# modelscope/FunASR

Hardware: AMD Instinct MI355X
Metric: audio-seconds/sec (RTF^-1) Paraformer-large 30s@bs64 (higher is better)
Workload: dtype f32 (GEMM / self-attention operands split into 2 fp16 planes, 3 fp16 MFMA products, f32 accumulate; all else f32)

## Files before the change

### funasr_amd/_lib.py

```python
from __future__ import annotations

import ctypes as C
import os
import subprocess
import threading

_HERE = os.path.dirname(os.path.abspath(__file__))
LIB_PATH = os.environ.get("PF_LIB_PATH") or os.path.join(_HERE, "libparaformer_hip.so")
CSRC_DIR = os.path.join(_HERE, "csrc")

ABI_VERSION = 5

_lock = threading.Lock()
_lib = None


class HipRuntimeError(RuntimeError):
    """A pf_* entry point returned a non-zero status."""


class pf_frontend_config(C.Structure):
    _fields_ = [
        ("sample_rate", C.c_int32), ("frame_length", C.c_int32), ("frame_shift", C.c_int32),
        ("n_mels", C.c_int32), ("lfr_m", C.c_int32), ("lfr_n", C.c_int32),
# ... 186 lines not shown
    "pf_conformer_set_tensor": (C.c_int, [_vp, C.c_char_p, _vp, _i64]),
    "pf_conformer_missing": (C.c_int, [_vp]),
    "pf_conformer_set_precision": (C.c_int, [_vp, _i32]),
    "pf_conformer_num_frames": (_i32, [_vp, _i32, _i32]),
    "pf_conformer_forward": (C.c_int, [_vp, _vp, _pi32, _i32, _i32, _vp, _pi32, _vp]),
    "pf_tfencoder_create": (_vp, [C.POINTER(pf_tfencoder_config)]),
    "pf_tfencoder_destroy": (None, [_vp]),
    "pf_tfencoder_set_tensor": (C.c_int, [_vp, C.c_char_p, _vp, _i64]),
    "pf_tfencoder_missing": (C.c_int, [_vp]),
    "pf_tfencoder_set_precision": (C.c_int, [_vp, _i32]),
    "pf_tfencoder_num_frames": (_i32, [_vp, _i32, _i32]),
    "pf_tfencoder_forward": (C.c_int, [_vp, _vp, _pi32, _i32, _i32, _vp, _pi32, _vp]),
    "pf_k_tf_attention": (C.c_int, [_vp, _vp, _i32, _i32, _i32, _vp, _vp]),
    "pf_k_tf_embed_rows": (C.c_int, [_vp, _i32, _vp, _i32, _i32, _i32, _f32, _vp, _vp]),
    "pf_tdecoder_create": (_vp, [C.POINTER(pf_tdecoder_config)]),
    "pf_tdecoder_destroy": (None, [_vp]),
    "pf_tdecoder_set_tensor": (C.c_int, [_vp, C.c_char_p, _vp, _i64]),
    "pf_tdecoder_missing": (C.c_int, [_vp]),
    "pf_tdecoder_begin": (C.c_int, [_vp, _vp, _i32, _i32, _i32, _vp]),
    "pf_tdecoder_step": (C.c_int, [_vp, _pi32, _i32, _i32, _vp, _vp]),
    "pf_tdecoder_reorder": (C.c_int, [_vp, _pi32, _i32, _vp]),
    "pf_fsmndecoder_create": (_vp, [C.POINTER(pf_fsmndecoder_config)]),
    "pf_fsmndecoder_destroy": (None, [_vp]),
    "pf_fsmndecoder_set_tensor": (C.c_int, [_vp, C.c_char_p, _vp, _i64]),
    "pf_fsmndecoder_missing": (C.c_int, [_vp]),
    "pf_fsmndecoder_begin": (C.c_int, [_vp, _vp, _i32, _i32, _i32, _vp]),
    "pf_fsmndecoder_step": (C.c_int, [_vp, _pi32, _i32, _i32, _vp, _vp]),
    "pf_fsmndecoder_reorder": (C.c_int, [_vp, _pi32, _i32, _vp]),
    "pf_k_fsmn_step": (C.c_int, [_vp, _vp, _vp, _vp, _vp, _vp, _vp, _vp, _i32, _i32, _i32, _i32, _i32, _vp, _vp, _f32, _vp, _vp, _vp]),
    "pf_k_cross_attention_step": (C.c_int, [_vp, _vp, _i32, _i32, _i32, _i32, _vp, _vp]),
    "pf_k_relpos_attention": (C.c_int, [_vp, _vp, _vp, _vp, _vp, _i32, _i32, _i32, _i32, _vp, _vp]),
    "pf_k_conformer_glu_dw": (C.c_int, [_vp, _vp, _vp, _vp, _vp, _i32, _i32, _i32, _i32, _vp, _vp]),
    "pf_transducer_create": (_vp, [C.POINTER(pf_transducer_config)]),
    "pf_transducer_destroy": (None, [_vp]),
    "pf_transducer_set_weights": (C.c_int, [_vp, C.c_char_p, _vp, _i64]),
    "pf_transducer_missing": (C.c_int, [_vp]),
    "pf_transducer_last_error": (C.c_char_p, [_vp]),
    "pf_transducer_search": (C.c_int, [_vp, _vp, _i32, _i32, _i32, _i32, _pi32, _pi32, C.POINTER(C.c_double), _i32, _pi32,
                                       C.POINTER(C.c_int64), _vp]),
    "pf_k_rnnt_pred_step": (C.c_int, [_vp, _vp, _vp, _vp, _vp, _i32, _i32, _i32, _i32, _i32, _i32, _i32, _i32, _i32, _vp]),
    "pf_k_rnnt_joint_partial_floats": (_i64, [_i32, _i32]),
    "pf_k_rnnt_joint_topk": (C.c_int, [_vp, _vp, _vp, _vp, _i32, _i32, _i32, _vp, _vp, _vp]),
    "pf_ctc_create": (_vp, [_i32, _i32]),
    "pf_ctc_destroy": (None, [_vp]),
    "pf_ctc_set_tensor": (C.c_int, [_vp, C.c_char_p, _vp, _i64]),
    "pf_ctc_missing": (C.c_int, [_vp]),
    "pf_ctc_greedy": (C.c_int, [_vp, _vp, _i32, _vp, _vp, _vp]),
    "pf_ctc_set_precision": (C.c_int, [_vp, _i32]),
    "pf_posterior_embed_create": (_vp, [_i32, _i32, _i32]),
    "pf_posterior_embed_destroy": (None, [_vp]),
    "pf_posterior_embed_set_tensor": (C.c_int, [_vp, C.c_char_p, _vp, _i64]),
    "pf_posterior_embed_missing": (C.c_int, [_vp]),
    "pf_posterior_embed_set_precision": (C.c_int, [_vp, _i32]),
    "pf_posterior_embed_set_chunk_rows": (C.c_int, [_vp, _i32]),
    "pf_posterior_embed_debug_poison": (C.c_int, [_vp, _i32]),
    "pf_posterior_embed_runs": (C.c_int, [_vp, _vp, _vp, _pi32, _i32, _i32, _pi32, _vp, _vp]),
    "pf_posterior_embed_embeds": (C.c_int, [_vp, _i32, _i32, _i32, _vp, _vp, _vp]),
    "pf_stream_create": (_vp, [_vp, _vp, _vp, C.POINTER(pf_stream_config)]),
    "pf_stream_destroy": (None, [_vp]),
    "pf_stream_set_pe": (C.c_int, [_vp, _vp, _i32]),
    "pf_stream_reset": (C.c_int, [_vp, _vp]),
    "pf_stream_set_option": (C.c_int, [_vp, C.c_char_p, _i32]),
    "pf_stream_step": (C.c_int, [_vp, _vp, _i32, _i32, _i32, _pi32, _pi32, _vp, _vp]),
    "pf_stream_step_begin": (C.c_int, [_vp, _vp, _i32, _i32, _i32, _vp, _vp]),
    "pf_stream_step_end": (C.c_int, [_vp, _pi32, _pi32]),
    "pf_stream_peek": (C.c_int, [_vp, _vp, _vp, _pi32]),
    "pf_frontend_fbank": (C.c_int, [_vp, _vp, _i64, _vp, _vp]),
    "pf_frontend_lfr_cmvn": (C.c_int, [_vp, _vp, _i32, _i32, _vp, _vp]),
    "pf_set_skinny_max_m": (C.c_int, [_i32]),
    "pf_measurement_build": (C.c_int, []),
    "pf_k_conv1d_gemm_f32": (C.c_int, [_vp, _vp, _vp, _vp, _i32, _i32, _i32, _i32, _i32, _i32, _i32, _vp, _vp]),
    "pf_k_gemm_f32": (C.c_int, [_vp, _i32, _vp, _i32, _vp, _vp, _i32, _vp, _i32, _vp, _i32, _i32, _i32, _i32, _i32, _vp]),
    "pf_k_gemm_bf16": (C.c_int, [_vp, _i32, _vp, _i32, _vp, _vp, _i32, _vp, _i32, _vp, _i32, _i32, _i32, _i32, _i32, _i32, _vp]),
    "pf_k_gemm_bf16_time": (C.c_int, [_vp, _i32, _vp, _i32, _vp, _vp, _i32, _i32, _i32, _i32, _i32, _i32, C.POINTER(C.c_float), _vp]),
    "pf_k_cast_bf16": (C.c_int, [_vp, _vp, _i64, _vp]),
    "pf_k_split3": (C.c_int, [_vp, _i32, _vp, _i32, _i64, _i32, _i32, _vp]),
    "pf_k_gemm_split3": (C.c_int, [_vp, _i32, _i64, _vp, _i32, _i64, _vp, _vp, _i32, _vp, _i32, _vp, _i32, _vp, _i32, _i64,
                                   _i32, _i32, _i32, _i32, _i32, C.POINTER(C.c_float), _vp]),
    "pf_k_split2": (C.c_int, [_vp, _i32, _vp, _i32, _i64, _i32, _i32, _f32, _vp]),
    "pf_k_gemm_f16x2": (C.c_int, [_vp, _i32, _i64, _vp, _i32, _i64, _f32, _vp, _vp, _i32, _vp, _i32, _vp, _i32, _vp, _i32, _i64,
                                  _f32, _i32, _i32, _i32, _i32, _i32, _i32, C.POINTER(C.c_float), _vp]),
    "pf_k_attention_f16x2": (C.c_int, [_vp, _i64, _vp, _i64, _vp, _i32, _i64, _vp, _i64, _vp, _i32, _i32, _i32, _i32, _f32, _f32,
                                       _i32, _i32, C.POINTER(C.c_float), _vp]),
    "pf_k_gemm_f16x2_row": (C.c_int, [_vp, _i32, _i64, _vp, _i32, _i64, _f32, _vp, _vp, _i32, _vp, _i32, _vp, _i32, _vp, _vp, _f32,
                                      _vp, _i64, _f32, _vp, _i32, _i32, _i32, _i32, _i32, C.POINTER(C.c_float), _vp]),
    "pf_k_gemm_skinny_ln": (C.c_int, [_vp, _i32, _vp, _i32, _vp, _vp, _i32, _vp, _i32, _i32, _i32, _i32, _i32, _vp, _vp, _vp, _vp, _f32, _vp, _vp, _vp, _vp]),
    "pf_k_ln_consts": (C.c_int, [_vp, _i32, _i32, _i32, _vp, _vp, _vp, _vp, _vp]),
    "pf_k_ffn_f16x2": (C.c_int, [_vp, _vp, _vp, _vp, _vp, _f32, _f32, _f32, _vp, _vp, _vp, _vp, _f32, _vp, _f32, _vp, _i32, _i32, _i32,
                                 C.POINTER(C.c_float), _vp]),
    "pf_k_gemm_f16x2_row_fsmn": (C.c_int, [_vp, _i32, _i64, _vp, _i32, _i64, _f32, _vp, _vp, _i32, _vp, _vp, _vp, _vp, _i32, _vp, _i32,
                                           _vp, _vp, _f32, _vp, _i64, _f32, _vp, _i32, _i32, _i32, _i32, C.POINTER(C.c_float), _vp]),
    "pf_k_layernorm_planes": (C.c_int, [_vp, _i32, _vp, _vp, _vp, _i32, _i64, _f32, _i32, _i32, _f32, _i32, C.POINTER(C.c_float), _vp]),
    "pf_k_gemm_f16x2_qkv": (C.c_int, [_vp, _i32, _i64, _vp, _i32, _i64, _f32, _vp, _i32, _i32, _i32, _i32, _vp, _vp, _i64, _vp, _vp,
                                      _i32, _i64, _f32, _f32, _f32, _i32, _i32, C.POINTER(C.c_float), _vp]),
    "pf_k_gemm_f16x2_argmax": (C.c_int, [_vp, _i32, _i64, _vp, _i32, _i64, _f32, _vp, _i32, _i32, _i32, _vp, _vp, _vp, _vp]),
    "pf_k_gemm_argmax_f32": (C.c_int, [_vp, _i32, _vp, _i32, _vp, _i32, _i32, _i32, _vp, _vp, _vp, _vp]),
    "pf_k_log_softmax": (C.c_int, [_vp, _i32, _vp, _i32, _i32, _i32, _vp]),
    "pf_k_layernorm": (C.c_int, [_vp, _i32, _vp, _vp, _vp, _i32, _i32, _i32, _i32, _f32, _vp]),
    "pf_k_fsmn": (C.c_int, [_vp, _i32, _vp, _vp, _i32, _vp, _i32, _vp, _i32, _i32, _i32, _i32, _i32, _vp]),
    "pf_k_attention_f32": (C.c_int, [_vp, _i32, _vp, _i32, _vp, _i32, _vp, _i32, _vp, _i32, _i32, _i32, _i32, _f32, _vp]),
    "pf_k_attention_f32_two_source": (C.c_int, [_vp, _i32, _vp, _i32, _vp, _i32, _vp, _i32, _vp, _i32, _vp, _i32, _vp, _i32,
                                                _i32, _i32, _i32, _i32, _i32, _i32, _f32, _vp]),
    "pf_k_attention_small": (C.c_int, [_vp, _i32, _vp, _i32, _vp, _i32, _vp, _i32, _vp, _i32, _i32, _i32, _i32, _i32, _f32, _vp]),
    "pf_k_gather_rows": (C.c_int, [_vp, _i32, _i32, _vp, _vp, _i32, _i32, _vp]),
    "pf_k_attention_split3": (C.c_int, [_vp, _i32, _vp, _i32, _vp, _i32, _vp, _i32, _vp, _i32, _i32, _i32, _i32, _f32, _vp]),
    "pf_k_attention_bf16": (C.c_int, [_vp, _i32, _vp, _i32, _vp, _i32, _vp, _i32, _vp, _i32, _i32, _i32, _i32, _f32, _vp]),
    "pf_k_lstm": (C.c_int, [_vp, _vp, _vp, _vp, _vp, _i32, _i32, _i32, _i32, _i32, _vp, _vp]),
    "pf_k_cif": (C.c_int, [_vp, _vp, _i32, _i32, _i32, _i32, _vp, _vp, _vp, _vp]),
    "pf_k_cif_tail": (C.c_int, [_vp, _vp, _vp, _i32, _i32, _i32, _i32, _f32, _i32, _i32, _vp, _vp, _vp, _vp, _vp, _vp]),
    "pf_k_ctc_runs": (C.c_int, [_vp, _pi32, _i32, _i32, _i32, _vp, _vp, _i32, _vp]),
    "pf_k_argmax_rows": (C.c_int, [_vp, _i32, _i32, _i32, _vp, _vp]),
    "pf_k_log_softmax_stats": (C.c_int, [_vp, _i32, _i32, _i32, _vp, _vp, _vp]),
    "pf_k_ctc_align_scratch_bytes": (_i64, [_i32, _i32, _i32]),
    "pf_k_ctc_align": (C.c_int, [_vp, _i32, _i32, _i32, _i32, _vp, _vp, _vp, _i32, _pi32, _pi32, _i32, _i32, _vp, _i32, _vp, _i64, _vp]),
    "pf_k_gemm_f32_time": (C.c_int, [_vp, _i32, _vp, _i32, _vp, _vp, _i32, _i32, _i32, _i32, _i32, C.POINTER(C.c_float), _vp]),
    "pf_dp_unique_id": (C.c_int, [_vp, _i32]),
    "pf_dp_create": (_vp, [_vp, _i32, _i32, _i32]),
    "pf_dp_destroy": (C.c_int, [_vp]),
    "pf_dp_world": (C.c_int, [_vp]),
    "pf_dp_rank": (C.c_int, [_vp]),
    "pf_dp_broadcast_encoder": (C.c_int, [_vp, _vp, _i32, _vp]),
    "pf_dp_broadcast_predictor": (C.c_int, [_vp, _vp, _i32, _vp]),
    "pf_dp_broadcast_decoder": (C.c_int, [_vp, _vp, _i32, _vp]),
    "pf_dp_broadcast_ctc": (C.c_int, [_vp, _vp, _i32, _vp]),
    "pf_paraformer_create": (_vp, [_vp, _vp, _vp]),
    "pf_paraformer_destroy": (None, [_vp]),
    "pf_paraformer_forward": (C.c_int, [_vp, _vp, _vp, _i32, _i32, _vp, _vp, _i32, _vp, _vp, _vp, _vp]),
    "pf_paraformer_begin": (C.c_int, [_vp, _vp, _vp, _i32, _i32, _vp, _vp]),
    "pf_paraformer_finish": (C.c_int, [_vp, _i32, _vp, _i32, _vp, _vp, _vp, _vp]),
    "pf_paraformer_encoder_out": (_vp, [_vp]),
    "pf_paraformer_embeds": (_vp, [_vp]),
    "pf_dp_gather_ids": (C.c_int, [_vp, _vp, _i64, _vp, _i32, _vp]),
    "pf_dp_broadcast_raw": (C.c_int, [_vp, _vp, _i64, _i32, _vp]),
    "pf_prof_enable": (C.c_int, [C.c_int]),
    "pf_prof_reset": (C.c_int, []),
    "pf_prof_read": (C.c_int, [C.c_int, C.POINTER(C.c_double), C.POINTER(C.c_double), C.POINTER(C.c_int64)]),
    "pf_prof_read_tags": (C.c_int, [C.c_int, C.POINTER(C.c_char_p), C.POINTER(C.c_int), C.POINTER(C.c_double), C.POINTER(C.c_double),
                                    C.POINTER(C.c_int64)]),
}


def build(verbose: bool = False) -> str:
    cmd = ["make", "-C", CSRC_DIR, "-j8"]
    res = subprocess.run(cmd, stdout=subprocess.PIPE, stderr=subprocess.STDOUT, text=True)
    if verbose:
        print(res.stdout)
    if res.returncode != 0:
        raise RuntimeError("building libparaformer_hip.so failed:\n" + res.stdout)
    return LIB_PATH


def load():
    global _lib
    with _lock:
        if _lib is not None:
            return _lib
        if not os.path.exists(LIB_PATH):
            raise ImportError(
                f"{LIB_PATH} not found: the HIP extension is the only implementation of this package. "
                f"Build it with `make -C {CSRC_DIR}` (or `python -c 'import __graft_entry__ as g; g.build()'`)."
            )
        lib = C.CDLL(LIB_PATH)
        for name, (res, args) in SIGNATURES.items():
            fn = getattr(lib, name)
            fn.restype = res
            fn.argtypes = args
# ... 22 lines not shown
```

### funasr_amd/csrc/attention_f16x2.hip

```cpp
#include "common.h"

namespace pf {

namespace {

constexpr int DK = 128, KT = 32;
constexpr int KP_B = KT * DK * 2;
constexpr int VP_B = DK * KT * 2;
constexpr int STAGE_B = 2 * KP_B + 2 * VP_B;
constexpr int OLD = DK + 4;
constexpr int SLAB_B = 8 * 32 * OLD * 4;
constexpr int LDS_BYTES = SLAB_B > 3 * STAGE_B ? SLAB_B : 3 * STAGE_B;
constexpr float P_SCALE = 1024.f;
typedef _Float16 f16x8 __attribute__((ext_vector_type(8)));

constexpr float LAZY_TAU = 3.0f;
template <int PIPE, bool LAZY = false>
__global__ __launch_bounds__(512, 2) void attention_f16x2_kernel(Attn2Args p) {
    extern __shared__ __attribute__((aligned(16))) unsigned char smem[];
    constexpr int NSTAGE = PIPE ? 3 : 2;
    constexpr int QB = 256;
    constexpr int NV = 1;

    const int tid = threadIdx.x, lane = tid & 63;
    const int wave = __builtin_amdgcn_readfirstlane(tid >> 6);
    const int hh = lane >> 5, idx = lane & 31;
    int b, head, qblk;
    if (p.xcd_nqb > 0) {
        const int L = blockIdx.x, j = L >> 3;
        const int pair = (j / p.xcd_nqb) * 8 + (L & 7);
        if (pair >= p.B * p.H) return;
        qblk = j % p.xcd_nqb; head = pair % p.H; b = pair / p.H;
    } else {
        b = blockIdx.z; head = blockIdx.y; qblk = blockIdx.x;
    }
    const int Tq = p.qoffs ? p.qoffs[b + 1] - p.qoffs[b] : (p.Tq > 0 ? p.Tq : p.Tp);
    if (qblk * QB >= Tq) return;
    const int q = qblk * QB + wave * 32 + idx;
    const int qc = q < Tq ? q : Tq - 1;
    const int klen = p.klens[b];
    const int kstart = p.koffs ? p.koffs[b] : b * p.Tp;
    const size_t row0 = (size_t)(kstart & ~15);
    const int kskip = kstart & 15, kend = kskip + klen;
    const size_t qrow0 = p.qoffs ? (size_t)p.qoffs[b] : (size_t)b * Tq;

    f16x8 qf[2][8];
    {
        const unsigned short* qp = p.Q + (qrow0 + qc) * p.ldq + head * DK + hh * 8;
#pragma unroll
        for (int pl = 0; pl < 2; ++pl)
#pragma unroll
            for (int s = 0; s < 8; ++s)
                qf[pl][s] = __builtin_bit_cast(f16x8, *reinterpret_cast<const uint4*>(qp + pl * p.q_plane + 16 * s));
    }

    floatx16 o[4];
#pragma unroll
    for (int d = 0; d < 4; ++d)
#pragma unroll
        for (int r = 0; r < 16; ++r) o[d][r] = 0.f;
    float m_run = -INFINITY, l_run = 0.f;

    const unsigned short* ksrc[NV];
    const unsigned short* vsrc[NV];
    unsigned lds_w[NV];
#pragma unroll
    for (int v = 0; v < NV; ++v) {
        const int vw = wave * NV + v;
        const int kr = vw * 4 + (lane >> 4);
        ksrc[v] = p.K + (row0 + kr) * p.ldk + head * DK + (((lane & 15) ^ (kr & 15)) * 8);
        const int dr = vw * 16 + (lane >> 2);
        vsrc[v] = p.VT + (size_t)(head * DK + dr) * p.ldvt + row0 + (((lane & 3) ^ ((dr >> 2) & 3)) * 8);
        lds_w[v] = __builtin_amdgcn_readfirstlane(lds_addr_of(smem) + (unsigned)vw * 1024);
    }
    auto stage = [&](int kt) {
        const size_t ko = (size_t)kt * KT * p.ldk;
#pragma unroll
        for (int v = 0; v < NV; ++v) {
            const unsigned base = lds_w[v] + (unsigned)(kt % NSTAGE) * STAGE_B;
            glds16(ksrc[v] + ko, base);
            glds16(ksrc[v] + p.k_plane + ko, base + KP_B);
            glds16(vsrc[v] + kt * KT, base + 2 * KP_B);
            glds16(vsrc[v] + p.vt_plane + kt * KT, base + 2 * KP_B + VP_B);
        }
    };

    const float sscale = p.sscale_dev ? p.sscale * *p.sscale_dev : p.sscale;
    const float sscale2 = LAZY ? sscale * 1.4426950408889634f : sscale;
#define PF_EXP(x_) (LAZY ? __builtin_amdgcn_exp2f(x_) : __expf(x_))
    constexpr float PSC = LAZY ? 1.f : P_SCALE;
    const int ntiles = (kend + KT - 1) / KT;

#define PF_QK(KT_, SA, SB)                                                                                            \
    {                                                                                                                 \
        const unsigned char* kp = smem + ((KT_) % NSTAGE) * STAGE_B + idx * 256;                                      \
        _Pragma("unroll") for (int r = 0; r < 16; ++r) { SA[r] = 0.f; SB[r] = 0.f; }                                  \
        _Pragma("unroll") for (int st = 0; st < 8; ++st) {                                                            \
            const int co = ((2 * st + hh) ^ (idx & 15)) * 16;                                                         \
            const f16x8 kh = __builtin_bit_cast(f16x8, *reinterpret_cast<const uint4*>(kp + co));                     \
            const f16x8 kl = __builtin_bit_cast(f16x8, *reinterpret_cast<const uint4*>(kp + KP_B + co));              \
            SA = __builtin_amdgcn_mfma_f32_32x32x16_f16(kl, qf[0][st], SA, 0, 0, 0);                                  \
            SB = __builtin_amdgcn_mfma_f32_32x32x16_f16(kh, qf[0][st], SB, 0, 0, 0);                                  \
            SA = __builtin_amdgcn_mfma_f32_32x32x16_f16(kh, qf[1][st], SA, 0, 0, 0);                                  \
        }                                                                                                             \
    }
#define PF_SOFTMAX(K0_, SA, SB)                                                                                       \
    {                                                                                                                 \
        float mx = -INFINITY;                                                                                         \
        if (LAZY && (K0_) >= kskip && (K0_) + KT <= kend) {         \
            _Pragma("unroll") for (int r = 0; r < 16; ++r) {                                                          \
                s[r] = (SA[r] + SB[r]) * sscale2;                                                                     \
// ... 48 lines not shown
    }

    float s[16];
    const bool active = qblk * QB + wave * 32 < Tq;
    if constexpr (PIPE == 0) {
        stage(0);
        for (int kt = 0; kt < ntiles; ++kt) {
            glds_wait_all();
            __syncthreads();
            if (kt + 1 < ntiles) stage(kt + 1);
            if (active) {
                floatx16 sa, sb;
                PF_QK(kt, sa, sb)
                PF_SOFTMAX(kt * KT, sa, sb)
                PF_PV(kt)
            }
        }
    } else {
        floatx16 ca, cb, na, nb;
        stage(0);
        if (ntiles > 1) stage(1);
        glds_wait_all();
        __syncthreads();
        PF_QK(0, ca, cb)
        for (int kt = 0; kt < ntiles; ++kt) {
            if (kt > 0) { glds_wait_all(); __syncthreads(); }
            if (kt + 2 < ntiles) stage(kt + 2);
            const int kn = kt + 1 < ntiles ? kt + 1 : kt;
            PF_QK(kn, na, nb)
            PF_SOFTMAX(kt * KT, ca, cb)
#pragma unroll
            for (int g = 0; g < 24; ++g) {
                __builtin_amdgcn_sched_group_barrier(0x008, 1, 0);
                __builtin_amdgcn_sched_group_barrier(0x002, 7, 0);
            }
            PF_PV(kt)
            ca = na; cb = nb;
        }
    }
#undef PF_QK
#undef PF_EXP
#undef PF_SOFTMAX
#undef PF_PV

    __syncthreads();
    float* slab = reinterpret_cast<float*>(smem) + wave * (32 * OLD);
    {
        const float inv = (LAZY ? p.oscale * P_SCALE : p.oscale) / l_run;
#pragma unroll
        for (int d = 0; d < 4; ++d)
#pragma unroll
            for (int g = 0; g < 4; ++g) {
                const float4 t = make_float4(o[d][4 * g + 0] * inv, o[d][4 * g + 1] * inv, o[d][4 * g + 2] * inv, o[d][4 * g + 3] * inv);
                *reinterpret_cast<float4*>(slab + idx * OLD + d * 32 + 8 * g + 4 * hh) = t;
            }
    }
    const int qw0 = qblk * QB + wave * 32;
#pragma unroll
    for (int it = 0; it < 8; ++it) {
        const int rr = it * 4 + (lane >> 4), c8 = (lane & 15) * 8;
        const float4 a = *reinterpret_cast<const float4*>(slab + rr * OLD + c8);
        const float4 c = *reinterpret_cast<const float4*>(slab + rr * OLD + c8 + 4);
        if (qw0 + rr < Tq) {
            uint4 h, l;
            split2_pk(a.x, a.y, h.x, l.x);
            split2_pk(a.z, a.w, h.y, l.y);
            split2_pk(c.x, c.y, h.z, l.z);
            split2_pk(c.z, c.w, h.w, l.w);
            unsigned short* op = p.O + (qrow0 + qw0 + rr) * p.ldo + head * DK + c8;
            *reinterpret_cast<uint4*>(op) = h;
            *reinterpret_cast<uint4*>(op + p.o_plane) = l;
        }
    }
}

}

int launch_attention_f16x2(const Attn2Args& a, hipStream_t stream) {
    PF_REQUIRE(a.B > 0 && a.H > 0 && (a.koffs || (a.Tp > 0 && a.Tp % 16 == 0)), "attention_f16x2: rows per sequence must be a positive multiple of 16");
    PF_REQUIRE(a.ldq % 8 == 0 && a.ldk % 8 == 0 && a.ldvt % 8 == 0 && a.ldo % 8 == 0 && a.q_plane % 8 == 0 &&
               a.k_plane % 8 == 0 && a.vt_plane % 8 == 0 && a.o_plane % 8 == 0, "attention_f16x2: strides % 8");
    PF_REQUIRE(((uintptr_t)a.Q & 15) == 0 && ((uintptr_t)a.K & 15) == 0 && ((uintptr_t)a.VT & 15) == 0 && ((uintptr_t)a.O & 15) == 0,
               "attention_f16x2: 16-B alignment");
    static PerDeviceOnce configured;
    if (!configured.done()) {
#if defined(PF_MEASUREMENT_KERNELS)
        PF_HIP_TRY(hipFuncSetAttribute(reinterpret_cast<const void*>(&attention_f16x2_kernel<0>),
                                       hipFuncAttributeMaxDynamicSharedMemorySize, LDS_BYTES));
        PF_HIP_TRY(hipFuncSetAttribute(reinterpret_cast<const void*>(&attention_f16x2_kernel<1>),
                                       hipFuncAttributeMaxDynamicSharedMemorySize, LDS_BYTES));
#endif
        PF_HIP_TRY(hipFuncSetAttribute(reinterpret_cast<const void*>(&attention_f16x2_kernel<0, true>),
                                       hipFuncAttributeMaxDynamicSharedMemorySize, LDS_BYTES));
        configured.mark();
    }
    const int rows = a.Tq > 0 ? a.Tq : a.Tp;
    Attn2Args k = a;
#if defined(PF_MEASUREMENT_KERNELS)
    PF_REQUIRE(a.variant == 0 || a.variant == 1 || a.variant == 3, "attention_f16x2: variant must be 0, 1 or 3");
#else
    PF_REQUIRE(a.variant == 3, "attention_f16x2: variant must be 3 (variants 0 / 1: the measurement library, make measure)");
#endif
    const int nqb = ceil_div(rows, 256);
    dim3 grid(nqb, a.H, a.B);
    k.xcd_nqb = (a.xcd_nqb >= 0 && nqb > 1) ? nqb : 0;
    if (k.xcd_nqb > 0) grid = dim3((unsigned)(ceil_div(a.B * a.H, 8) * 8 * nqb), 1, 1);
    if (a.variant == 3)
        hipLaunchKernelGGL((attention_f16x2_kernel<0, true>), grid, dim3(512), LDS_BYTES, stream, k);
#if defined(PF_MEASUREMENT_KERNELS)
    else if (a.variant == 1)
        hipLaunchKernelGGL(attention_f16x2_kernel<1>, grid, dim3(512), LDS_BYTES, stream, k);
    else
        hipLaunchKernelGGL(attention_f16x2_kernel<0>, grid, dim3(512), LDS_BYTES, stream, k);
#endif
    PF_HIP_TRY(hipGetLastError());
    return 0;
}

}
```

### funasr_amd/csrc/common.h

```cpp
#pragma once
#include <hip/hip_runtime.h>
#include <stdint.h>
#include <stdio.h>
#include <string>
#include <atomic>

typedef float floatx16 __attribute__((ext_vector_type(16)));
typedef float floatx4 __attribute__((ext_vector_type(4)));

namespace pf {

inline int current_device_slot() {
    int d = 0;
    if (hipGetDevice(&d) != hipSuccess || d < 0) d = 0;
    return d & 63;
}
struct PerDeviceOnce {
    std::atomic<bool> flag[64];
    PerDeviceOnce() { for (auto& f : flag) f.store(false, std::memory_order_relaxed); }
    bool done() const { return flag[current_device_slot()].load(std::memory_order_acquire); }
    void mark() { flag[current_device_slot()].store(true, std::memory_order_release); }
};
inline int device_cu_count() {
    static std::atomic<int> n[64];
    const int slot = current_device_slot();
    int v = n[slot].load(std::memory_order_relaxed);
    if (v > 0) return v;
    int dev = 0;
    hipDeviceProp_t pr;
    v = 256;
    if (hipGetDevice(&dev) == hipSuccess && hipGetDeviceProperties(&pr, dev) == hipSuccess && pr.multiProcessorCount > 0) v = pr.multiProcessorCount;
    n[slot].store(v, std::memory_order_relaxed);
    return v;
}


void set_error(const std::string& msg);
const char* get_error();

#define PF_HIP_TRY(expr)                                                         \
    do {                                                                         \
        hipError_t _e = (expr);                                                  \
        if (_e != hipSuccess) {                                                  \
            pf::set_error(std::string(#expr) + ": " + hipGetErrorString(_e));    \
            return -2;                                                           \
        }                                                                        \
    } while (0)

#define PF_REQUIRE(cond, msg)                                                    \
    do {                                                                         \
        if (!(cond)) {                                                           \
            pf::set_error(std::string("invalid argument: ") + (msg));            \
            return -1;                                                           \
        }                                                                        \
    } while (0)

static inline int ceil_div(int a, int b) { return (a + b - 1) / b; }

__device__ __forceinline__ float wave_sum(float v) {
#pragma unroll
    for (int o = 32; o > 0; o >>= 1) v += __shfl_xor(v, o, 64);
    return v;
}
__device__ __forceinline__ float wave_max(float v) {
#pragma unroll
    for (int o = 32; o > 0; o >>= 1) v = fmaxf(v, __shfl_xor(v, o, 64));
    return v;
}

__device__ __forceinline__ unsigned short f32_to_bf16(float f) {
    unsigned int u = __builtin_bit_cast(unsigned int, f);
    u += 0x7fffu + ((u >> 16) & 1u);
    return (unsigned short)(u >> 16);
}
__device__ __forceinline__ float bf16_to_f32(unsigned short h) {
    return __builtin_bit_cast(float, (unsigned int)h << 16);
}

__device__ __forceinline__ void split3(float x, unsigned short& h, unsigned short& m, unsigned short& l) {
    h = f32_to_bf16(x);
    const float r1 = x - bf16_to_f32(h);
    m = f32_to_bf16(r1);
    const float r2 = r1 - bf16_to_f32(m);
    l = f32_to_bf16(r2);
}
typedef __bf16 pf_bf16x2 __attribute__((ext_vector_type(2)));
typedef float pf_floatx2 __attribute__((ext_vector_type(2)));
// ... 214 lines not shown
};
bool ffn_f16x2_applicable(int D, int F);
int launch_ffn_f16x2(const FfnArgs& a, hipStream_t stream);
int launch_gemm_f16x2_row8(const GemmRowArgs& a, int bm, hipStream_t stream);
bool gemm_f16x2_row_applicable(int N, int K);
int launch_gemm_f16x2_row(const GemmRowArgs& a, hipStream_t stream);
int launch_split2(const float* x, int ldx, unsigned short* y, int ldy, size_t plane, int M, int N, float scale,
                  hipStream_t stream, const float* scale_dev = nullptr, int seq_out = 0, int seq_in = 0);
int launch_kv_scales(const float* amax_dev, const float* l1_bmax_dev, int n_layers, float* out, hipStream_t stream);
int launch_pow2_scale(const float* amax_dev, float* sc, hipStream_t stream);
int launch_absmax(const float* x, size_t n, float* out_dev, hipStream_t stream);
int launch_rowl1_bound(const float* W, int rows, int cols, int ld, const float* bias, float in_bound, float* out_dev,
                       hipStream_t stream);

int launch_splitk_reduce_ln(const float* part, int slices, size_t slice_stride, int M, int D, const float* bias, int relu, const float* R1, int ldr1,
                            const float* R2, int ldr2, float* C, int ldc, const float* gamma, const float* beta, float eps, float* y, int ldy, int out_mode,
                            size_t plane, float oscale, hipStream_t stream);
int launch_layernorm(const float* x, int ldx, const float* gamma, const float* beta, float* y, int ldy,
                     int M, int D, int Dpad, float eps, hipStream_t stream, int out_mode = 0, int in_bf16 = 0,
                     size_t plane = 0, float oscale = 1.f, int seq_out = 0, int seq_in = 0, const int* out_map = nullptr);

int launch_scale_cols(float* x, int ld, int M, int N, float sc, hipStream_t stream);
int launch_log_softmax(const float* x, int ldx, float* y, int ldy, int M, int N, hipStream_t stream);
int launch_log_softmax_stats(const float* x, int ldx, int M, int N, float* lse, int* pred, hipStream_t stream);
int launch_scale_add_pe(const float* x, const float* pe, float* y, int B, int T, int D, float scale,
                        hipStream_t stream, int Tp = 0);
int launch_scale_add_pe_rows(const float* x, const float* pe, float* y, const int* map, int M, int T, int D, float scale,
                             hipStream_t stream);

struct FsmnArgs {
    const float* in;  int ldin;
    const float* w;
    const float* R;   int ldr;
    float* out;       int ldo;
    const int* lens;
    int B, T, C, K, left_pad;
    int in_bf16;
    const int* offs;
};
int launch_fsmn(const FsmnArgs& a, hipStream_t stream);

struct AttnArgs {
    const float* Q; int ldq;
    const float* K; int ldk;
    const float* V; int ldv;
    float* O;       int ldo;
    const int* klens;
    int B, H, Tq, Tk;
    float scale;
    const float* K2; int ldk2;
    const float* V2; int ldv2;
    int T2, n2;
    const int* n1_dev; int n1_stride;
    unsigned short* O3; size_t o_plane;
    int few_q;
    int app_rows, app_r0; const int* app_wp; int app_wp_stride; const int* app_gate;
    int app_mod;
    int mask_mode; const int* vad_pos;
    const float* fs_in; int fs_ldin; const float* fs_w; float* fs_out; int fs_ldo; int fs_T;
    unsigned short* O2; int ldo2; size_t o2_plane; float o2_scale;
};
inline bool attention_takes_fewq(const AttnArgs& a) { return a.few_q && a.Tq <= 32 && !a.O3; }
inline bool attention_fuses_append(const AttnArgs& a) {
    return a.few_q && a.Tq <= 16 && !a.O3 && a.K2 && a.app_rows > 0 && (a.app_rows < a.Tk ? a.app_rows : a.Tk) <= 16;
}
int launch_attention_f32(const AttnArgs& a, hipStream_t stream);
int launch_attention_bf16(const AttnArgs& a, hipStream_t stream);
int launch_attention_split3(const AttnArgs& a, hipStream_t stream);
struct Attn2Args {
    const unsigned short* Q; int ldq; size_t q_plane;
    const unsigned short* K; int ldk; size_t k_plane;
    const unsigned short* VT; int ldvt; size_t vt_plane;
    unsigned short* O; int ldo; size_t o_plane;
    const int* klens;
    int B, H, Tp;
    int Tq;
    float sscale;
    const float* sscale_dev;
    float oscale;
    int variant;
    const int* qoffs;
    int xcd_nqb;
    const int* koffs;
};
int launch_attention_f16x2(const Attn2Args& a, hipStream_t stream);

int launch_asf_scores(const float* Q, int ldq, const float* K, int ldk, float* P_scratch, float* out, int H, int dk, int N, int T,
                      int klen, float scale, hipStream_t stream);
bool attention_small_applicable(const AttnArgs& a, int dk);
int launch_attention_small(const AttnArgs& a, int dk, hipStream_t stream);
int launch_scatter_i32(const int* in, const int* map, int* out, int n, hipStream_t stream);
int launch_gather_rows(const float* table, int ld, int rows, const int* ids, float* out, int n, int D, hipStream_t stream);

int launch_vad_fsmn(const float* x, int ldx, const float* w, const float* cache_in, float* cache_out, float* y, int ldy,
                    int B, int T, int C, int L, int S, hipStream_t stream);
int launch_vad_softmax_sil(const float* x, int ldx, int M, int N, const int* ids, int n_ids, float* p_sil, float* probs,
                           int ldp, hipStream_t stream);
int launch_frame_decibel(const float* wav, int n_frames, int flen, int shift, float* out, hipStream_t stream);

int launch_kws_fsmn(const float* x, int ldx, const float* wl, const float* wr, float* y, int ldy, int B, int T, int C, int L, int LS,
                    int R, int RS, hipStream_t stream);
int launch_kws_candidates(const float* x, long ldx, int M, int V, const unsigned* mask, int* out, hipStream_t stream);

}
```

### funasr_amd/csrc/engine_decoder.hip

```cpp
#include "engine_internal.h"

namespace pf {

static std::string dec_layer_prefix(bool contextual, int n_blocks, int i) {
    return (contextual && i == n_blocks - 1) ? std::string("last_decoder.") : "decoders." + std::to_string(i) + ".";
}
static std::string dec2_layer_prefix(int i) { return "decoders2." + std::to_string(i) + "."; }

static int dec_layer_add(TensorTable& tt, const pf_decoder_config& c, const std::string& p, int kind) {
    const int D = c.d_model, F = c.ffn_dim;
    int rc = 0;
    rc |= tt.add(p + "norm1.weight", D);
    rc |= tt.add(p + "norm1.bias", D);
    rc |= tt.add(p + "feed_forward.w_1.weight", (int64_t)F * D);
    rc |= tt.add(p + "feed_forward.w_1.bias", F);
    rc |= tt.add(p + "feed_forward.norm.weight", F);
    rc |= tt.add(p + "feed_forward.norm.bias", F);
    rc |= tt.add(p + "feed_forward.w_2.weight", (int64_t)D * F);
    if (kind >= DEC_FFN_FSMN) {
        rc |= tt.add(p + "norm2.weight", D);
        rc |= tt.add(p + "norm2.bias", D);
        rc |= tt.add(p + "self_attn.fsmn_block.weight", (int64_t)D * c.kernel_size);
    }
    if (kind >= DEC_FFN_FSMN_ATTN) {
// ... 342 lines not shown
    int rc = 0;
    for (int i = 0; i < c.n_blocks; ++i) rc |= dec_layer_add(d->tt, c, dec_layer_prefix(contextual, c.n_blocks, i), DEC_FFN_FSMN_ATTN);
    if (contextual) {
        rc |= d->tt.add("bias_decoder.norm3.weight", D);
        rc |= d->tt.add("bias_decoder.norm3.bias", D);
        rc |= d->tt.add("bias_decoder.src_attn.linear_q.weight", (int64_t)D * D);
        rc |= d->tt.add("bias_decoder.src_attn.linear_q.bias", D);
        rc |= d->tt.add("bias_decoder.src_attn.linear_k_v.weight", (int64_t)2 * D * D);
        rc |= d->tt.add("bias_decoder.src_attn.linear_k_v.bias", 2 * D);
        rc |= d->tt.add("bias_decoder.src_attn.linear_out.weight", (int64_t)D * D);
        rc |= d->tt.add("bias_decoder.src_attn.linear_out.bias", D);
        rc |= d->tt.add("bias_output.weight", (int64_t)D * 2 * D);
    }
    rc |= dec_layer_add(d->tt, c, "decoders3.0.", DEC_FFN);
    rc |= d->tt.add("after_norm.weight", D);
    rc |= d->tt.add("after_norm.bias", D);
    if (c.vocab_size > 0) {
        rc |= d->tt.add("output_layer.weight", (int64_t)c.vocab_size * D);
        rc |= d->tt.add("output_layer.bias", c.vocab_size);
    }
    if (rc) return nullptr;
    return reinterpret_cast<pf_decoder*>(d.release());
}

static int decoder_forward_impl(Decoder* d, const float* memory, const int32_t* mem_lens, const float* embeds,
                                const int32_t* tok_lens, int32_t B, int32_t T, int32_t N, float* logits, int32_t* ids,
                                float* hidden_out, hipStream_t s, int asf_layer, float* asf_scores, const DecCtxArgs* cx = nullptr) {
    PF_REQUIRE(d && memory && mem_lens && embeds && tok_lens && B > 0 && T > 0 && N > 0, "decoder_forward: null/empty");
    for (int b = 0; b < B; ++b) {
        PF_REQUIRE(mem_lens[b] >= 1 && mem_lens[b] <= T, "decoder_forward: memory lens out of range");
        PF_REQUIRE(tok_lens[b] >= 0 && tok_lens[b] <= N, "decoder_forward: token lens out of range");
    }
    PF_REQUIRE(d->precision == 0 || d->cfg.d_model / d->cfg.n_heads == 128, "decoder_forward: heads of d_k <= 64 exist in the fp32 mode only");
    int rc;
    if ((rc = decoder_prepare(d, d->precision == 3 && asf_layer < 0 && !cx, s))) return rc;
    const pf_decoder_config& c = d->cfg;
    const int D = c.d_model, F = c.ffn_dim, V = c.vocab_size;
    int Mq = B * N;
    const int Mq_pad = B * N, Mk = B * T;
    if (d->x.ensure(sizeof(float) * (size_t)Mq * D) || d->t1.ensure(sizeof(float) * (size_t)Mq * D) ||
        d->t2.ensure(sizeof(float) * (size_t)Mq * D) || d->ffn.ensure(sizeof(float) * (size_t)Mq * F) ||
        d->ffn2.ensure(sizeof(float) * (size_t)Mq * F) || d->q.ensure(sizeof(float) * (size_t)Mq * D) ||
        d->kv.ensure(sizeof(float) * (size_t)Mk * 2 * D) || d->ctx.ensure(sizeof(float) * (size_t)Mq * D) ||
        d->hid.ensure(sizeof(float) * (size_t)Mq * D))
        return -2;
    if ((rc = upload_lens(d->mem_lens, mem_lens, B, s))) return rc;
    if ((rc = upload_lens(d->tok_lens, tok_lens, B, s))) return rc;
    float* x = d->x.as<float>();
    float* t1 = d->t1.as<float>();
    float* t2 = d->t2.as<float>();
    const bool may_pack = d->precision == 3 && asf_layer < 0 && !cx && ids && !logits && !hidden_out && V > 0;
    if (!may_pack) PF_HIP_TRY(hipMemcpyAsync(x, embeds, sizeof(float) * (size_t)Mq * D, hipMemcpyDeviceToDevice, s));
    if (V == 0 && asf_layer < 0) PF_REQUIRE(!logits && !ids && hidden_out && d->precision != 1,
                           "decoder_forward: a decoder without output layer returns hidden states only (fp32 / bf16x3)");
    PF_REQUIRE(d->contextual == (cx != nullptr) || asf_layer >= 0, "decoder_forward: a contextual decoder runs through pf_decoder_forward_contextual");
    if (d->precision == 1 && !logits && asf_layer < 0 && !cx) return decoder_forward_bf16(d, memory, B, T, N, ids, hidden_out, s);
    const bool x3 = d->precision == 2 && asf_layer < 0 && !cx;
    const bool x2 = d->precision == 3 && asf_layer < 0 && !cx;
    const int Tp = round_up(T, 16), Mkp = B * Tp;
    double mem_rows = 0, tok_mem = 0;
    for (int b = 0; b < B; ++b) { mem_rows += mem_lens[b]; tok_mem += (double)mem_lens[b] * tok_lens[b]; }
    const unsigned short* mem3 = nullptr;
    const unsigned short* mem2 = nullptr;
    float* dsc = nullptr;
    if (x2) {
        const size_t cap_k = d->k2.cap, cap_v = d->vt2.cap;
        if (d->t16.ensure(sizeof(unsigned short) * 2 * (size_t)Mq * D) || d->ffn16.ensure(sizeof(unsigned short) * 2 * (size_t)Mq * F) ||
            d->q16.ensure(sizeof(unsigned short) * 2 * (size_t)Mq * D) || d->ctx16.ensure(sizeof(unsigned short) * 2 * (size_t)Mq * D) ||
            d->mem16.ensure(sizeof(unsigned short) * 2 * (size_t)Mkp * D) || d->dsc.ensure(sizeof(float) * 4) ||
            d->k2.ensure(sizeof(unsigned short) * 2 * ((size_t)Mkp + 32) * D) || d->vt2.ensure(sizeof(unsigned short) * 2 * D * ((size_t)Mkp + 64)) ||
            d->dscl.ensure(sizeof(float) * 4 * c.n_blocks))
            return -2;
        if (d->k2.cap != cap_k) PF_HIP_TRY(hipMemsetAsync(d->k2.p, 0, d->k2.cap, s));
        if (d->vt2.cap != cap_v) PF_HIP_TRY(hipMemsetAsync(d->vt2.p, 0, d->vt2.cap, s));
        dsc = d->dsc.as<float>();
        if ((rc = launch_absmax(memory, (size_t)Mk * D, dsc, s))) return rc;
        if ((rc = launch_pow2_scale(dsc, dsc + 1, s))) return rc;
        if ((rc = launch_kv_scales(dsc, d->dlb.as<float>(), c.n_blocks, d->dscl.as<float>(), s))) return rc;
        if ((rc = launch_split2(memory, D, d->mem16.as<unsigned short>(), D, (size_t)Mkp * D, Mkp, D, 1.f, s, dsc + 1, Tp, T))) return rc;
        mem2 = d->mem16.as<unsigned short>();
    }
    bool pack = false;
    const int* offs_dev = nullptr;
    if (may_pack) {
        int total = 0;
        d->h_offs.assign((size_t)B + 1, 0);
        for (int b = 0; b < B; ++b) { d->h_offs[b] = total; total += tok_lens[b]; }
        d->h_offs[B] = total;
        if (total > 0 && total < Mq_pad) {
            d->h_map.resize((size_t)total);
            for (int b = 0; b < B; ++b) for (int t = 0; t < tok_lens[b]; ++t) d->h_map[(size_t)d->h_offs[b] + t] = b * N + t;
            if (d->offs_dev.ensure(sizeof(int32_t) * ((size_t)B + 1)) || d->map_dev.ensure(sizeof(int32_t) * (size_t)Mq_pad) ||
                d->ids_packed.ensure(sizeof(int32_t) * (size_t)Mq_pad)) return -2;
            if (upload_h2d(d->offs_dev.p, d->h_offs.data(), sizeof(int32_t) * ((size_t)B + 1), s) ||
                upload_h2d(d->map_dev.p, d->h_map.data(), sizeof(int32_t) * (size_t)total, s)) return -2;
            if ((rc = launch_gather_rows(embeds, D, Mq_pad, d->map_dev.as<int>(), x, total, D, s))) return rc;
            pack = true; offs_dev = d->offs_dev.as<int>(); Mq = total;
        }
    }
    if (may_pack && !pack) PF_HIP_TRY(hipMemcpyAsync(x, embeds, sizeof(float) * (size_t)Mq * D, hipMemcpyDeviceToDevice, s));
    if (x3) {
        if (d->t16.ensure(sizeof(unsigned short) * 3 * (size_t)Mq * D) || d->mem16.ensure(sizeof(unsigned short) * 3 * (size_t)Mk * D))
            return -2;
        if ((rc = launch_split3(memory, D, d->mem16.as<unsigned short>(), D, (size_t)Mk * D, Mk, D, s))) return rc;
        mem3 = d->mem16.as<unsigned short>();
    }
    DecRows rows{x2 ? 3 : x3 ? 2 : 0, Mq, B, N, offs_dev, (c.kernel_size - 1) / 2 + (c.sanm_shift > 0 ? c.sanm_shift : 0), s};
    for (int l = 0; l < c.n_blocks; ++l) {
        const DecLayerW& w = d->layers[l];
        if ((rc = dec_block_step(d, w, x, rows))) return rc;
        if (x2) {
            unsigned short* t2p = d->t16.as<unsigned short>();
            {
                ProfScope ps(PROF_LN, 8.0 * Mq * (double)D, s);
                if ((rc = launch_layernorm(x, D, w.n3g, w.n3b, reinterpret_cast<float*>(t2p), D, Mq, D, D, c.ln_eps, s, 3, 0,
                                           (size_t)Mq * D, pow2f(w.e_n3)))) return rc;
            }
            Gemm2Args g{};
            g.A = t2p; g.lda = D; g.a_plane = (size_t)Mq * D; g.W = w.q_2; g.ldw = D; g.w_plane = (size_t)D * D;
            g.oscale = pow2f(-(w.e_n3 + w.ew_q)); g.bias = w.q_b; g.C2 = d->q16.as<unsigned short>(); g.ldc2 = D;
            g.c_plane = (size_t)Mq * D; g.cscale = powf((float)(D / c.n_heads), -0.5f) * pow2f(w.e_q);
            g.M = Mq; g.N = D; g.K = D;
            ProfScope ps(PROF_GEMM3, 2.0 * Mq * (double)D * D, s);
            if ((rc = launch_gemm_f16x2(g, s))) return rc;
        } else {
            if ((rc = layernorm(x, D, w.n3g, w.n3b, t1, D, Mq, D, D, c.ln_eps, s))) return rc;
            if ((rc = gemm_simple(t1, D, w.q_w, D, w.q_b, d->q.as<float>(), D, Mq, D, D, 0, nullptr, 0, nullptr, 0, s)))
                return rc;
        }
        if (x2) {
            const float* lsc = d->dscl.as<float>() + 4 * l;
            unsigned short* k2 = d->k2.as<unsigned short>();
            unsigned short* vt2 = d->vt2.as<unsigned short>();
            {
                Gemm2Args g{};
                g.A = mem2; g.lda = D; g.a_plane = (size_t)Mkp * D; g.W = w.kv_2; g.ldw = D; g.w_plane = (size_t)2 * D * D;
                g.oscale = pow2f(-w.ew_kv); g.oscale_dev = dsc + 2; g.bias = w.kv_b; g.M = Mkp; g.N = 2 * D; g.K = D;
                g.qkv_D = D; g.kv_form = 1; g.Kp = k2; g.qk_plane = ((size_t)Mkp + 32) * D; g.VT = vt2; g.ldvt = Mkp + 64;
                g.vt_plane = (size_t)D * (Mkp + 64); g.k_mul = 1.f; g.v_mul = 1.f; g.kv_mul_dev = lsc;
                ProfScope ps(PROF_GEMM3, 2.0 * mem_rows * 2.0 * D * D, s);
                if ((rc = launch_gemm_f16x2(g, s))) return rc;
            }
            {
                Attn2Args aa{};
                aa.Q = d->q16.as<unsigned short>(); aa.ldq = D; aa.q_plane = (size_t)Mq * D;
                aa.K = k2; aa.ldk = D; aa.k_plane = ((size_t)Mkp + 32) * D; aa.VT = vt2; aa.ldvt = Mkp + 64;
                aa.vt_plane = (size_t)D * (Mkp + 64); aa.O = d->ctx16.as<unsigned short>(); aa.ldo = D; aa.o_plane = (size_t)Mq * D;
                aa.klens = d->mem_lens.as<int>(); aa.B = B; aa.H = c.n_heads; aa.Tp = Tp; aa.Tq = N; aa.qoffs = offs_dev;
                aa.sscale = pow2f(-w.e_q); aa.sscale_dev = lsc + 2; aa.oscale = pow2f(-10);
                aa.variant = 3;
                ProfScope ps(PROF_ATTN, 4.0 * tok_mem * D, s);
                if ((rc = launch_attention_f16x2(aa, s))) return rc;
            }
            if ((rc = gemm2_simple(d->ctx16.as<unsigned short>(), D, Mq, 0, w.o_2, w.ew_o, w.o_b, x, D, D, D, 0, x, D, s, lsc + 3)))
                return rc;
            continue;
        } else if (x3) {
            if ((rc = gemm3_simple(mem3, D, Mk, d->tt.get_split3(w.prefix + "src_attn.linear_k_v.weight", 2 * D, D, s), w.kv_b,
                                   d->kv.as<float>(), 2 * D, 2 * D, D, 0, s))) return rc;
        } else if ((rc = gemm_simple(memory, D, w.kv_w, D, w.kv_b, d->kv.as<float>(), 2 * D, Mk, 2 * D, D, 0, nullptr, 0,
                                     nullptr, 0, s))) return rc;
        const bool ctx_block = cx && l == c.n_blocks - 1;
        if (ctx_block) {
            if (d->xself.ensure(sizeof(float) * (size_t)Mq * D) || d->xcat.ensure(sizeof(float) * (size_t)Mq * 2 * D)) return -2;
            PF_HIP_TRY(hipMemcpyAsync(d->xself.p, x, sizeof(float) * (size_t)Mq * D, hipMemcpyDeviceToDevice, s));
        }
        if (l == asf_layer) {
            if (d->asf_p.ensure(sizeof(float) * (size_t)c.n_heads * N * T)) return -2;
            return launch_asf_scores(d->q.as<float>(), D, d->kv.as<float>(), 2 * D, d->asf_p.as<float>(), asf_scores, c.n_heads,
                                     D / c.n_heads, N, T, mem_lens[0], powf((float)(D / c.n_heads), -0.5f), s);
        }
        AttnArgs aa{};
        aa.Q = d->q.as<float>(); aa.ldq = D; aa.K = d->kv.as<float>(); aa.ldk = 2 * D;
        aa.V = d->kv.as<float>() + D; aa.ldv = 2 * D; aa.O = d->ctx.as<float>(); aa.ldo = D;
        aa.klens = d->mem_lens.as<int>(); aa.B = B; aa.H = c.n_heads; aa.Tq = N; aa.Tk = T;
        aa.scale = powf((float)(D / c.n_heads), -0.5f);
        if ((rc = attention(aa, 4.0 * B * (double)N * T * D, s, false, D / c.n_heads))) return rc;
        if (ctx_block) {
            float* xcat = d->xcat.as<float>();
            const float* xs = d->xself.as<float>();
            if ((rc = gemm_simple(d->ctx.as<float>(), D, w.o_w, D, w.o_b, xcat, 2 * D, Mq, D, D, 0, nullptr, 0, nullptr, 0, s)))
                return rc;
            const int Mh = B * cx->n_hot;
            if (d->kv.ensure(sizeof(float) * (size_t)(Mh > Mk ? Mh : Mk) * 2 * D)) return -2;
            std::vector<int32_t> hl((size_t)B, cx->n_hot);
            if ((rc = upload_lens(d->ctx_lens, hl.data(), B, s))) return rc;
            PF_HIP_TRY(hipStreamSynchronize(s));
            if ((rc = layernorm(xs, D, d->tt.get("bias_decoder.norm3.weight"), d->tt.get("bias_decoder.norm3.bias"), t1, D, Mq, D, D,
                                c.ln_eps, s))) return rc;
            if ((rc = gemm_simple(t1, D, d->tt.get("bias_decoder.src_attn.linear_q.weight"), D,
                                  d->tt.get("bias_decoder.src_attn.linear_q.bias"), d->q.as<float>(), D, Mq, D, D, 0, nullptr, 0, nullptr, 0, s))) return rc;
            if ((rc = gemm_simple(cx->info, D, d->tt.get("bias_decoder.src_attn.linear_k_v.weight"), D,
                                  d->tt.get("bias_decoder.src_attn.linear_k_v.bias"), d->kv.as<float>(), 2 * D, Mh, 2 * D, D, 0, nullptr, 0,
                                  nullptr, 0, s))) return rc;
            AttnArgs ab{};
            ab.Q = d->q.as<float>(); ab.ldq = D; ab.K = d->kv.as<float>(); ab.ldk = 2 * D; ab.V = d->kv.as<float>() + D; ab.ldv = 2 * D;
            ab.O = d->ctx.as<float>(); ab.ldo = D; ab.klens = d->ctx_lens.as<int>(); ab.B = B; ab.H = c.n_heads; ab.Tq = N; ab.Tk = cx->n_hot;
            ab.scale = aa.scale;
            if ((rc = attention(ab, 4.0 * B * (double)N * cx->n_hot * D, s))) return rc;
            if ((rc = gemm_simple(d->ctx.as<float>(), D, d->tt.get("bias_decoder.src_attn.linear_out.weight"), D,
                                  d->tt.get("bias_decoder.src_attn.linear_out.bias"), xcat + D, 2 * D, Mq, D, D, 0, nullptr, 0, nullptr, 0, s)))
                return rc;
            if (cx->clas_scale != 1.0f && (rc = launch_scale_cols(xcat + D, 2 * D, Mq, D, cx->clas_scale, s))) return rc;
            if ((rc = gemm_simple(xcat, 2 * D, d->tt.get("bias_output.weight"), 2 * D, nullptr, x, D, Mq, D, 2 * D, 0, nullptr, 0, xs, D, s)))
                return rc;
            continue;
        }
        if ((rc = gemm_simple(d->ctx.as<float>(), D, w.o_w, D, w.o_b, x, D, Mq, D, D, 0, nullptr, 0, x, D, s)))
            return rc;
    }
    rows.left_pad = (c.kernel_size - 1) / 2;
    for (const DecLayerW& w : d->layers2) if ((rc = dec_block_step(d, w, x, rows))) return rc;
    if ((rc = dec_ffn_rows(d, d->last, x, t2, rows))) return rc;
    float* hid = hidden_out ? hidden_out : d->hid.as<float>();
    if (x2 && V > 0 && ids && !logits && !hidden_out) {
        int ew_v = 0;
        const unsigned short* wv2 = d->tt.get_split2("output_layer.weight", V, D, &ew_v, s);
        if (!wv2) return -2;
        unsigned short* h2 = d->t16.as<unsigned short>();
        {
            ProfScope ps(PROF_LN, 8.0 * Mq * (double)D, s);
            if ((rc = launch_layernorm(t2, D, d->tt.get("after_norm.weight"), d->tt.get("after_norm.bias"), reinterpret_cast<float*>(h2), D,
                                       Mq, D, D, c.ln_eps, s, 3, 0, (size_t)Mq * D, pow2f(d->e_an)))) return rc;
        }
        if (argmax_scratch(d->pval, d->pidx, Mq, gemm_f16x2_argmax_parts(Mq, V))) return -2;
        rc = argmax_f16x2(h2, D, (size_t)Mq * D, wv2, D, (size_t)V * D, pow2f(-(d->e_an + ew_v)), nullptr, d->tt.get("output_layer.bias"),
                          Mq, V, D, d->pval.as<float>(), d->pidx.as<int>(), pack ? d->ids_packed.as<int>() : ids, s);
        if (rc || !pack) return rc;
        PF_HIP_TRY(hipMemsetAsync(ids, 0, sizeof(int32_t) * (size_t)Mq_pad, s));
        return launch_scatter_i32(d->ids_packed.as<int>(), d->map_dev.as<int>(), ids, Mq, s);
    }
    if ((rc = layernorm(t2, D, d->tt.get("after_norm.weight"), d->tt.get("after_norm.bias"), hid, D, Mq, D, D,
                        c.ln_eps, s))) return rc;
// ... 118 lines not shown
```

### funasr_amd/csrc/engine_internal.h

```cpp
#pragma once
#include <math.h>
#include <string.h>

#include <cmath>
#include <map>
#include <memory>
#include <mutex>
#include <string>
#include <vector>

#include "../../include/paraformer_hip.h"
#include "cif.h"
#include "lstm.h"
#include "common.h"
#include "frontend.h"
#include "stream.h"
#include "engine_tables.h"


namespace pf {

void set_error(const std::string& msg);
const char* get_error();

// ... 365 lines not shown
    return e > 15 ? 15 : e;
}
static inline float pow2f(int e) { return ldexpf(1.f, e); }

static inline bool encoder_w2_row_form(const Encoder* e, int M) {
    if (e->w2_row != 2) return e->w2_row == 1;
    const int n_cu = device_cu_count();
    const int blocks = ceil_div(M, 256) * (e->cfg.d_model / 256), rounds = ceil_div(blocks, n_cu);
    return !(e->cfg.d_model % 256 == 0 && blocks >= (int)(0.65 * rounds * n_cu));
}

void note_concurrent_streams();

struct EncChunkCtx {
    float* ring; int cap; const StreamDev* st; int append_rows;
    const int* lens;
    int mod = 0;
    bool x2 = false;
    float* ln_stats = nullptr;
    bool ln_in_ready = false;
    const float* ln_c_qkv = nullptr;
    const float* ln_c_w1 = nullptr;
    const EncLayerW* x2_out_next = nullptr;
    bool x2_in_ready = false;
    int x2_short_k = 0;
    bool x2_fold = false;
    bool x2_attn_planes = false;
    bool fsmn_rides = false;
    const EncLayerW* next = nullptr;
};

struct Predictor {
    pf_predictor_config cfg;
    TensorTable tt;
    DevBuf col, conv, zero_row;
    struct CifState { DevBuf lens, alphas, peaks, rems, flags, nfires, curs, ntok; int B = 0, T = 0; } st[2];
    bool v3 = false;
    pf_predictor_v3_config c3{};
    DevBuf up, x_tm, pre, lstm_out, h_a, h_b, cell, tok_dev, ulens, pack, ts_lens;
    unsigned long long packed_for = TensorTable::NOT_PREPARED;
    std::vector<int32_t> ul_host;
};

int predictor_alphas_enqueue(Predictor* p, int slot, const float* hidden, const int32_t* lens_host, int B, int T, hipStream_t s);
const int32_t* predictor_counts_dev(Predictor* p, int slot);
const float* predictor_alphas_dev(Predictor* p, int slot);
const float* predictor_peaks_dev(Predictor* p, int slot);
int predictor_embeds_slot(Predictor* p, int slot, const float* hidden, int B, int T, int N, float* embeds, hipStream_t s);

enum { DEC_FFN = 0, DEC_FFN_FSMN = 1, DEC_FFN_FSMN_ATTN = 2 };
struct DecLayerW {
    std::string prefix;
    int kind = DEC_FFN;
    const float *n1g = nullptr, *n1b = nullptr, *w1 = nullptr, *b1 = nullptr, *fng = nullptr, *fnb = nullptr, *w2 = nullptr;
    const float *n2g = nullptr, *n2b = nullptr, *fsmn_w = nullptr;
    const float *n3g = nullptr, *n3b = nullptr, *q_w = nullptr, *q_b = nullptr, *kv_w = nullptr, *kv_b = nullptr, *o_w = nullptr,
        *o_b = nullptr;
    const unsigned short *w1_2 = nullptr, *w2_2 = nullptr, *q_2 = nullptr, *kv_2 = nullptr, *o_2 = nullptr;
    int ew_1 = 0, ew_2 = 0, ew_q = 0, ew_kv = 0, ew_o = 0, e_n1 = 0, e_fn = 0, e_n3 = 0, e_q = 0;
    float kv_l1b[4] = {0.f, 0.f, 0.f, 0.f};
};


struct Decoder {
    pf_decoder_config cfg;
    bool contextual = false;
    DevBuf xself, xcat, ctx_lens;
    TensorTable tt;
    std::vector<DecLayerW> layers;
    int n_blocks2 = 0;
    std::vector<DecLayerW> layers2;
    DecLayerW last;
    unsigned long long resolved_for = TensorTable::NOT_PREPARED, x2_for = TensorTable::NOT_PREPARED;
    DevBuf x, t1, t2, ffn, ffn2, q, kv, ctx, mem_lens, tok_lens, pval, pidx, hid;
    int precision = 0;
    DevBuf t16, ffn16, ffn2_16, q16, kv16, ctx16, mem16, hid16;
    DevBuf dsc;
    DevBuf dscl, dlb;
    DevBuf k2, vt2;
    DevBuf splitk;
    int e_an = 0;
    DevBuf asf_p;
    DevBuf offs_dev, map_dev, ids_packed;
    std::vector<int32_t> h_offs, h_map;
};


struct Ctc {
    int d_model, vocab;
    TensorTable tt;
    DevBuf pval, pidx;
    int precision = 0;
    DevBuf h2, dsc;
};

struct Stream {
    Encoder* e = nullptr; Predictor* p = nullptr; Decoder* d = nullptr;
    pf_stream_config cfg{};
    int S = 1, keep = 5, Wmax = 0, Nmax = 0, enc_cap = 0, dec_cap = 0, pe_rows = 0;
    int enc_mod = 0;
    DevBuf dev_state, cache_feats, feats_in, win, enc_ring, dec_ring, dec_fsmn, cif_hidden, cif_alpha, dec_valid, dec_wp,
        n_fired, pe, lensW, enc_out, embeds, ids, alphas;
    int32_t* h_ids = nullptr; int32_t* h_n = nullptr;
    hipStream_t stream = nullptr;
    hipEvent_t ev = nullptr;
    int start_idx = 0;
    std::map<int, hipGraphExec_t> graphs;
    std::map<int, int> seen;
    unsigned long long graph_epoch = 0;
    bool use_graph = true;
    bool x2 = false;
    int ln_carry = 2;
    bool fsmn_rides = true;
    DevBuf ln_stats;
    bool pending = false; int pending_rows = 0;
    bool wide_k = false;
    DevBuf ws_part, ws_count;
    DevBuf ln_consts;
    unsigned long long ln_ver_e = TensorTable::NOT_PREPARED, ln_ver_d = TensorTable::NOT_PREPARED;
    DevBuf dec_ln_a, dec_ln_b, dec_ln_f;
    int short_k = 3;
    bool ln_folded = true;
    DevBuf kvcat_w, kvcat_b, kvcat_2;
    int kvcat_e = 0;
    bool kv_batched = true;
    unsigned long long ver_e = TensorTable::NOT_PREPARED, ver_d = TensorTable::NOT_PREPARED;
    int e_mem = 0;
    std::vector<int> e_ctx;
    DevBuf mem2;
    ~Stream() {
        for (auto& kv : graphs) (void)hipGraphExecDestroy(kv.second);
        if (h_ids) (void)hipHostFree(h_ids);
        if (h_n) (void)hipHostFree(h_n);
        if (ev) (void)hipEventDestroy(ev);
        if (stream) (void)hipStreamDestroy(stream);
    }
};

struct Vad {
    pf_vad_config cfg;
    TensorTable tt;
    DevBuf a, b, c, cache_tmp, ids;
    size_t zeroed_for = 0;
};
static inline int vad_pad(int k) { return round_up(k, 32); }
struct LstmW { const float* w_ih[2]; const float* w_hh; const float* b_ih; const float* b_hh; };
struct DecCtxArgs { const float* info; int n_hot; float clas_scale; };

int check_device();
int upload_h2d(void* dst, const void* src, size_t bytes, hipStream_t s);
int upload_lens(DevBuf& buf, const int32_t* host, int B, hipStream_t s);
int gemm(const GemmArgs& a, hipStream_t s);
int gemm_simple(const float* A, int lda, const float* W, int ldw, const float* bias, float* C, int ldc,
                       int M, int N, int K, int relu, const float* R1, int ldr1, const float* R2, int ldr2,
                       hipStream_t s);
int layernorm(const float* x, int ldx, const float* g, const float* b, float* y, int ldy, int M, int D,
                     int Dpad, float eps, hipStream_t s);
int fsmn(const FsmnArgs& a, hipStream_t s);
int attention(const AttnArgs& a, double flops, hipStream_t s, bool x3 = false, int dk = 128, bool* appended = nullptr);
int frontend_upload_tables(Frontend* f, const std::vector<float>& window, const std::vector<float>& mel);
int frontend_default_tables(Frontend* f);
int encoder_prepare(Encoder* e, int mode, hipStream_t s);
int encoder_default_pe(Encoder* e, int T, hipStream_t s);
int encoder_block(Encoder* e, const EncLayerW& w, float* x_in, int ld_in, float* x, int B, int T,
                         hipStream_t s, const EncChunkCtx* cc = nullptr, bool xn_ready = false, const EncLayerW* next = nullptr);
int decoder_prepare(Decoder* d, bool x2, hipStream_t s);
int vocab_project(const float* hidden, int M, int D, const float* W, const float* bias, int V, float* logits,
// ... 42 lines not shown
```

### funasr_amd/csrc/engine_kernels.hip

```cpp
#include "ctc_align.h"
#include "engine_internal.h"

using namespace pf;

extern "C" {

int pf_k_gemm_skinny_ln(const float* A, int32_t lda, const float* W, int32_t ldw, const float* bias, const float* R2, int32_t ldr2,
                        float* Cout, int32_t ldc, int32_t M, int32_t N, int32_t K, int32_t relu, float* stats_out,
                        const float* stats_in, const float* ln_g, const float* ln_c, float ln_eps, const float* out_gamma, float* ws_part,
                        int32_t* ws_count, void* stream) {
    GemmArgs g{};
    g.ws_part = ws_part; g.ws_count = ws_count; g.ln_c1 = ln_c; g.ln_c2 = ln_c ? ln_c + N : nullptr; g.out_gamma = out_gamma;
    g.A = A; g.lda = lda; g.W = W; g.ldw = ldw; g.bias = bias; g.R2 = R2; g.ldr2 = ldr2; g.C = Cout; g.ldc = ldc;
    g.M = M; g.N = N; g.K = K; g.relu = relu; g.ln_stats_out = stats_out; g.ln_stats_in = stats_in; g.ln_g = ln_g; g.ln_eps = ln_eps;
    PF_REQUIRE(gemm_skinny_applicable(g), "gemm_skinny_ln: K % 16");
    return launch_gemm_skinny(g, reinterpret_cast<hipStream_t>(stream));
}
int pf_k_ln_consts(const float* W, int32_t ldw, int32_t N, int32_t K, const float* gamma, const float* beta, const float* bias, float* c,
                   void* stream) {
    return launch_ln_consts(W, ldw, N, K, gamma, beta, bias, c, c + N, reinterpret_cast<hipStream_t>(stream));
}
int pf_set_skinny_max_m(int32_t m) { g_skinny_max_m = m; return 0; }

int pf_k_gemm_f32(const float* A, int32_t lda, const float* W, int32_t ldw, const float* bias, const float* R1,
// ... 41 lines not shown
    for (int i = 0; i < iters; ++i) if ((rc = launch_gemm_f32(g, s))) return rc;
    PF_HIP_TRY(hipEventRecord(b, s));
    PF_HIP_TRY(hipEventSynchronize(b));
    float ms = 0.f;
    PF_HIP_TRY(hipEventElapsedTime(&ms, a, b));
    (void)hipEventDestroy(a);
    (void)hipEventDestroy(b);
    *ms_out = ms / iters;
    return 0;
}
int pf_k_split3(const float* x, int32_t ldx, void* y3, int32_t ldy, int64_t plane, int32_t M, int32_t N, void* stream) {
    return launch_split3(x, ldx, reinterpret_cast<unsigned short*>(y3), ldy, (size_t)plane, M, N,
                         reinterpret_cast<hipStream_t>(stream));
}
int pf_k_gemm_split3(const void* A3, int32_t lda, int64_t a_plane, const void* W3, int32_t ldw, int64_t w_plane,
                     const float* bias, const float* R1, int32_t ldr1, const float* R2, int32_t ldr2, float* C,
                     int32_t ldc, void* C3, int32_t ldc3, int64_t c_plane, int32_t M, int32_t N, int32_t K,
                     int32_t relu, int32_t iters, float* ms_out, void* stream) {
    hipStream_t s = reinterpret_cast<hipStream_t>(stream);
    Gemm3Args g{};
    g.A = reinterpret_cast<const unsigned short*>(A3); g.lda = lda; g.a_plane = (size_t)a_plane;
    g.W = reinterpret_cast<const unsigned short*>(W3); g.ldw = ldw; g.w_plane = (size_t)w_plane;
    g.bias = bias; g.R1 = R1; g.ldr1 = ldr1; g.R2 = R2; g.ldr2 = ldr2; g.C = C; g.ldc = ldc;
    g.C3 = reinterpret_cast<unsigned short*>(C3); g.ldc3 = ldc3; g.c_plane = (size_t)c_plane;
    g.M = M; g.N = N; g.K = K; g.relu = relu;
    int rc;
    if (iters <= 0 || !ms_out) return launch_gemm_split3(g, s);
    for (int i = 0; i < 3; ++i) if ((rc = launch_gemm_split3(g, s))) return rc;
    hipEvent_t a, b;
    PF_HIP_TRY(hipEventCreate(&a));
    PF_HIP_TRY(hipEventCreate(&b));
    PF_HIP_TRY(hipEventRecord(a, s));
    for (int i = 0; i < iters; ++i) if ((rc = launch_gemm_split3(g, s))) return rc;
    PF_HIP_TRY(hipEventRecord(b, s));
    PF_HIP_TRY(hipEventSynchronize(b));
    float ms = 0.f;
    PF_HIP_TRY(hipEventElapsedTime(&ms, a, b));
    (void)hipEventDestroy(a);
    (void)hipEventDestroy(b);
    *ms_out = ms / iters;
    return 0;
}
int pf_k_split2(const float* x, int32_t ldx, void* y2, int32_t ldy, int64_t plane, int32_t M, int32_t N, float scale,
                void* stream) {
    return launch_split2(x, ldx, reinterpret_cast<unsigned short*>(y2), ldy, (size_t)plane, M, N, scale,
                         reinterpret_cast<hipStream_t>(stream));
}
int pf_k_gemm_f16x2(const void* A2, int32_t lda, int64_t a_plane, const void* W2, int32_t ldw, int64_t w_plane,
                    float oscale, const float* bias, const float* R1, int32_t ldr1, const float* R2, int32_t ldr2,
                    float* C, int32_t ldc, void* C2, int32_t ldc2, int64_t c_plane, float cscale, int32_t M, int32_t N,
                    int32_t K, int32_t relu, int32_t tile, int32_t iters, float* ms_out, void* stream) {
    hipStream_t s = reinterpret_cast<hipStream_t>(stream);
    Gemm2Args g{};
    g.A = reinterpret_cast<const unsigned short*>(A2); g.lda = lda; g.a_plane = (size_t)a_plane;
    g.W = reinterpret_cast<const unsigned short*>(W2); g.ldw = ldw; g.w_plane = (size_t)w_plane; g.oscale = oscale;
    g.bias = bias; g.R1 = R1; g.ldr1 = ldr1; g.R2 = R2; g.ldr2 = ldr2; g.C = C; g.ldc = ldc;
    g.C2 = reinterpret_cast<unsigned short*>(C2); g.ldc2 = ldc2; g.c_plane = (size_t)c_plane; g.cscale = cscale;
    g.M = M; g.N = N; g.K = K; g.relu = relu; g.tile = tile & 0xfff;
    if (tile & 0x1000) { g.a_kstep = (long)M * 32; g.w_kstep = (long)N * 32; }
    if (tile & 0x2000) { g.w_kstep = (long)N * 32; g.ldw = 32; g.lda = K; }
    if (tile & 0x4000) { g.a_kstep = (long)M * 32; g.lda = 32; g.ldw = K; }
    static DevBuf splitk_scratch;
    if (tile & 0x8000) {
        if (splitk_scratch.ensure(sizeof(float) * 4 * (size_t)M * N)) return -2;
        g.ksplit = 4; g.part = splitk_scratch.as<float>();
    }
    int rc;
    if (iters <= 0 || !ms_out) return launch_gemm_f16x2(g, s);
    for (int i = 0; i < 3; ++i) if ((rc = launch_gemm_f16x2(g, s))) return rc;
    hipEvent_t a, b;
    PF_HIP_TRY(hipEventCreate(&a));
    PF_HIP_TRY(hipEventCreate(&b));
    PF_HIP_TRY(hipEventRecord(a, s));
    for (int i = 0; i < iters; ++i) if ((rc = launch_gemm_f16x2(g, s))) return rc;
    PF_HIP_TRY(hipEventRecord(b, s));
    PF_HIP_TRY(hipEventSynchronize(b));
    float ms = 0.f;
    PF_HIP_TRY(hipEventElapsedTime(&ms, a, b));
    (void)hipEventDestroy(a);
    (void)hipEventDestroy(b);
    *ms_out = ms / iters;
    return 0;
}
int pf_k_attention_f16x2(const void* Q2, int64_t q_plane, const void* K2, int64_t k_plane, const void* VT2, int32_t ldvt,
                         int64_t vt_plane, void* O2, int64_t o_plane, const int32_t* klens_dev, int32_t B, int32_t H,
                         int32_t Tp, int32_t Tq, float sscale, float oscale, int32_t variant, int32_t iters, float* ms_out,
                         void* stream) {
    hipStream_t s = reinterpret_cast<hipStream_t>(stream);
    Attn2Args aa{};
    const int D = H * 128;
    aa.Q = reinterpret_cast<const unsigned short*>(Q2); aa.ldq = D; aa.q_plane = (size_t)q_plane;
    aa.K = reinterpret_cast<const unsigned short*>(K2); aa.ldk = D; aa.k_plane = (size_t)k_plane;
    aa.VT = reinterpret_cast<const unsigned short*>(VT2); aa.ldvt = ldvt; aa.vt_plane = (size_t)vt_plane;
    aa.O = reinterpret_cast<unsigned short*>(O2); aa.ldo = D; aa.o_plane = (size_t)o_plane;
    aa.klens = klens_dev; aa.B = B; aa.H = H; aa.Tp = Tp; aa.Tq = Tq; aa.sscale = sscale; aa.oscale = oscale;
    aa.variant = variant & 15; aa.xcd_nqb = (variant & 16) ? -1 : 0;
    int rc;
    if (iters <= 0 || !ms_out) return launch_attention_f16x2(aa, s);
    for (int i = 0; i < 3; ++i) if ((rc = launch_attention_f16x2(aa, s))) return rc;
    hipEvent_t a, b;
    PF_HIP_TRY(hipEventCreate(&a));
    PF_HIP_TRY(hipEventCreate(&b));
    PF_HIP_TRY(hipEventRecord(a, s));
    for (int i = 0; i < iters; ++i) if ((rc = launch_attention_f16x2(aa, s))) return rc;
    PF_HIP_TRY(hipEventRecord(b, s));
    PF_HIP_TRY(hipEventSynchronize(b));
    float ms = 0.f;
    PF_HIP_TRY(hipEventElapsedTime(&ms, a, b));
    (void)hipEventDestroy(a);
    (void)hipEventDestroy(b);
    *ms_out = ms / iters;
    return 0;
}
int pf_k_gemm_f16x2_row(const void* A2, int32_t lda, int64_t a_plane, const void* W2, int32_t ldw, int64_t w_plane, float oscale,
                        const float* bias, const float* R1, int32_t ldr1, const float* R2, int32_t ldr2, float* C, int32_t ldc,
                        const float* ln_g, const float* ln_b, float ln_eps, void* Y2, int64_t y_plane, float yscale, float* Yf,
                        int32_t M, int32_t K, int32_t relu, int32_t a_nt, int32_t iters, float* ms_out, void* stream) {
    hipStream_t s = reinterpret_cast<hipStream_t>(stream);
    GemmRowArgs g{};
    g.A = reinterpret_cast<const unsigned short*>(A2); g.lda = lda; g.a_plane = (size_t)a_plane;
    g.W = reinterpret_cast<const unsigned short*>(W2); g.ldw = ldw; g.w_plane = (size_t)w_plane; g.oscale = oscale;
    g.bias = bias; g.R1 = R1; g.ldr1 = ldr1; g.R2 = R2; g.ldr2 = ldr2; g.C = C; g.ldc = ldc;
    g.ln_g = ln_g; g.ln_b = ln_b; g.ln_eps = ln_eps; g.Y2 = reinterpret_cast<unsigned short*>(Y2); g.ldy2 = 512;
    g.y_plane = (size_t)y_plane; g.yscale = yscale; g.Yf = Yf; g.ldyf = 512; g.M = M; g.N = 512; g.K = K; g.relu = relu;
    g.a_nt = a_nt & 3; g.block_rows = a_nt >> 8;
    if (iters <= 0 || !ms_out) return launch_gemm_f16x2_row(g, s);
    return time_launches([&] { return launch_gemm_f16x2_row(g, s); }, iters, ms_out, s);
}
#if defined(PF_MEASUREMENT_KERNELS)
int pf_k_ffn_f16x2(const void* X2, const void* W1, const void* W2, const float* b1, const float* b2, float oscale1, float hscale,
                   float oscale2, const float* R, float* Cout, const float* ln_g, const float* ln_b, float ln_eps, void* Y2,
                   float yscale, float* Yf, int32_t M, int32_t F, int32_t iters, float* ms_out, void* stream) {
    hipStream_t s = reinterpret_cast<hipStream_t>(stream);
    FfnArgs g{};
    g.abl = (F >> 24) & 15;
    const bool wkb = (F >> 28) & 1;
    F &= 0xffffff;
    g.X2 = reinterpret_cast<const unsigned short*>(X2); g.ldx = 512; g.x_plane = (size_t)M * 512;
    g.W1 = reinterpret_cast<const unsigned short*>(W1); g.ldw1 = 512; g.w1_plane = (size_t)F * 512;
    g.W2 = reinterpret_cast<const unsigned short*>(W2); g.ldw2 = F; g.w2_plane = (size_t)512 * F;
    g.b1 = b1; g.b2 = b2; g.oscale1 = oscale1; g.hscale = hscale; g.oscale2 = oscale2; g.R = R; g.ldr = 512; g.C = Cout; g.ldc = 512;
    g.ln_g = ln_g; g.ln_b = ln_b; g.ln_eps = ln_eps; g.Y2 = reinterpret_cast<unsigned short*>(Y2); g.ldy2 = 512;
    g.y_plane = (size_t)M * 512; g.yscale = yscale; g.Yf = Yf; g.ldyf = 512; g.M = M; g.D = 512; g.F = F;
    if (wkb) { g.ldw1 = 32; g.w1_kstep = (size_t)F * 32; g.ldw2 = 32; g.w2_kstep = (size_t)512 * 32; }
    if (iters <= 0 || !ms_out) return launch_ffn_f16x2(g, s);
    return time_launches([&] { return launch_ffn_f16x2(g, s); }, iters, ms_out, s);
}
#else
int pf_k_ffn_f16x2(const void* X2, const void* W1, const void* W2, const float* b1, const float* b2, float oscale1, float hscale,
                   float oscale2, const float* R, float* Cout, const float* ln_g, const float* ln_b, float ln_eps, void* Y2,
                   float yscale, float* Yf, int32_t M, int32_t F, int32_t iters, float* ms_out, void* stream) {
    set_error("pf_k_ffn_f16x2: the one-launch feed-forward is in the measurement library only (make -C funasr_amd/csrc measure)");
    return -1;
}
#endif
int pf_k_gemm_f16x2_row_fsmn(const void* A2, int32_t lda, int64_t a_plane, const void* W2, int32_t ldw, int64_t w_plane, float oscale,
                             const float* bias, const float* fs_v, int32_t ldfv, const float* fs_w, const int32_t* fs_lo,
                             const int32_t* fs_hi, const float* R2, int32_t ldr2, float* C, int32_t ldc, const float* ln_g,
                             const float* ln_b, float ln_eps, void* Y2, int64_t y_plane, float yscale, float* Yf, int32_t M, int32_t K,
                             int32_t a_nt, int32_t iters, float* ms_out, void* stream) {
    hipStream_t s = reinterpret_cast<hipStream_t>(stream);
    GemmRowArgs g{};
    g.A = reinterpret_cast<const unsigned short*>(A2); g.lda = lda; g.a_plane = (size_t)a_plane;
    g.W = reinterpret_cast<const unsigned short*>(W2); g.ldw = ldw; g.w_plane = (size_t)w_plane; g.oscale = oscale;
    g.bias = bias; g.fs_v = fs_v; g.ldfv = ldfv; g.fs_w = fs_w; g.fs_lo = fs_lo; g.fs_hi = fs_hi; g.R2 = R2; g.ldr2 = ldr2;
    g.C = C; g.ldc = ldc; g.ln_g = ln_g; g.ln_b = ln_b; g.ln_eps = ln_eps; g.Y2 = reinterpret_cast<unsigned short*>(Y2); g.ldy2 = 512;
    g.y_plane = (size_t)y_plane; g.yscale = yscale; g.Yf = Yf; g.ldyf = 512; g.M = M; g.N = 512; g.K = K;
    g.a_nt = a_nt & 3; g.block_rows = a_nt >> 8;
    if (iters <= 0 || !ms_out) return launch_gemm_f16x2_row(g, s);
    return time_launches([&] { return launch_gemm_f16x2_row(g, s); }, iters, ms_out, s);
}
int pf_k_layernorm_planes(const float* x, int32_t ldx, const float* gamma, const float* beta, void* y2, int32_t ldy, int64_t plane,
                          float scale, int32_t M, int32_t D, float eps, int32_t iters, float* ms_out, void* stream) {
    hipStream_t s = reinterpret_cast<hipStream_t>(stream);
    auto fn = [&] { return launch_layernorm(x, ldx, gamma, beta, reinterpret_cast<float*>(y2), ldy, M, D, ldy, eps, s, 3, 0, (size_t)plane, scale); };
    if (iters <= 0 || !ms_out) return fn();
    return time_launches(fn, iters, ms_out, s);
}
int pf_k_gemm_f16x2_qkv(const void* A2, int32_t lda, int64_t a_plane, const void* W2, int32_t ldw, int64_t w_plane, float oscale,
                        const float* bias, int32_t M, int32_t D, int32_t K, int32_t kv_form, void* Qp, void* Kp, int64_t qk_plane,
                        float* Vf, void* VT, int32_t ldvt, int64_t vt_plane, float q_mul, float k_mul, float v_mul, int32_t tile,
                        int32_t iters, float* ms_out, void* stream) {
    hipStream_t s = reinterpret_cast<hipStream_t>(stream);
    Gemm2Args g{};
    g.A = reinterpret_cast<const unsigned short*>(A2); g.lda = lda; g.a_plane = (size_t)a_plane;
    g.W = reinterpret_cast<const unsigned short*>(W2); g.ldw = ldw; g.w_plane = (size_t)w_plane; g.oscale = oscale; g.bias = bias;
    g.C = Vf; g.ldc = D; g.M = M; g.N = (kv_form ? 2 : 3) * D; g.K = K; g.qkv_D = D; g.kv_form = kv_form;
    g.Qp = reinterpret_cast<unsigned short*>(Qp); g.Kp = reinterpret_cast<unsigned short*>(Kp); g.qk_plane = (size_t)qk_plane;
    g.VT = reinterpret_cast<unsigned short*>(VT); g.ldvt = ldvt; g.vt_plane = (size_t)vt_plane;
    g.q_mul = q_mul; g.k_mul = k_mul; g.v_mul = v_mul; g.tile = tile;
    if (iters <= 0 || !ms_out) return launch_gemm_f16x2(g, s);
    return time_launches([&] { return launch_gemm_f16x2(g, s); }, iters, ms_out, s);
}
int pf_k_gemm_f16x2_argmax(const void* A2, int32_t lda, int64_t a_plane, const void* W2, int32_t ldw, int64_t w_plane, float oscale,
                           const float* bias, int32_t M, int32_t N, int32_t K, int32_t* ids, float* sval, int32_t* sidx,
// ... 222 lines not shown
```

### funasr_amd/csrc/gemm_f16x2.hip

```cpp
#include "common.h"
#include <cstdlib>
#include <type_traits>
#include "gemm_f16x2_epilogue.h"

namespace pf {

namespace {

typedef _Float16 f16x8 __attribute__((ext_vector_type(8)));

template <int WM, int WN, int WGM = 4, int KS_ = 32> struct Geo2 {
    static constexpr int NW = WGM * 2;
    static constexpr int BM = WGM * WM * 32, BN = 2 * WN * 32;
    static constexpr int KS = KS_, ROWB = 2 * KS, CPR = ROWB / 16, RPP = 1024 / ROWB;
    static constexpr int SWZ = CPR == 4 ? 2 : 3;
    static constexpr int A_PLANE_B = BM * ROWB, B_PLANE_B = BN * ROWB;
    static constexpr int STAGE_B = 2 * (A_PLANE_B + B_PLANE_B);
    static constexpr int NSTG = KS == 16 ? (WGM == 4 ? (163840 / STAGE_B > 6 ? 6 : 163840 / STAGE_B) : 3) : 2;
    static constexpr int NPIECE = STAGE_B / 1024;
    static constexpr int A_PIECES = 2 * BM / RPP;
    static constexpr int PPW = NPIECE / NW;
    static constexpr int ELD = WN * 32 + 4;
    static constexpr int SLAB_B = NW * 32 * ELD * 4;
    static constexpr int LDS_B = NSTG * STAGE_B > SLAB_B ? NSTG * STAGE_B : SLAB_B;
// ... 204 lines not shown
            PF_LOAD(0)
            {
#define a a1
#define b b1
                PF_LOAD(1)
#undef a
#undef b
            }
            if constexpr (SCHED == 2) { PF_PIECE(0); PF_PIECE(1); PF_PIECE(2); PF_PIECE(3); }
            PF_PROD(1, 0); if constexpr (SCHED == 1) { PF_PIECE(0); PF_PIECE(1); } else { PF_PIECE(4); PF_PIECE(5); }
            PF_PROD(0, 1); if constexpr (SCHED == 1) { PF_PIECE(2); PF_PIECE(3); } else { PF_PIECE(6); PF_PIECE(7); }
            PF_PROD(0, 0); if constexpr (SCHED == 1) { PF_PIECE(4); }
#define a a1
#define b b1
            PF_PROD(1, 0); if constexpr (SCHED == 1) { PF_PIECE(5); PF_PIECE(6); }
            PF_PROD(0, 1); if constexpr (SCHED == 1) { PF_PIECE(7); }
            PF_PROD(0, 0);
#undef a
#undef b
        }
#undef PF_PROD
#undef PF_LOAD
#undef PF_PIECE
    }
    }

    gemm2_epilogue<WM, WN, G::NW, MODE, OUT, ABL>(p, acc, smem, m0, n0, nblk, wave, wr, wc, lane);
}
template <int WM, int WN, int MODE, int OUT, int ABL = 0, int SCHED = 0, int WGM = 4, int KS_ = 32>
__global__ __launch_bounds__(WGM * 128, 2) void gemm_f16x2_kernel(Gemm2Args p, int nM, int nN) {
    typedef Geo2<WM, WN, WGM, KS_> G;
    constexpr int BM = G::BM, BN = G::BN;
    extern __shared__ __attribute__((aligned(16))) unsigned char smem[];

    const int L = blockIdx.x;
    const int xcd = L & 7, j8 = L >> 3;
    const int mblk = (j8 / nN) * 8 + xcd, nblk = j8 % nN;
    if (mblk >= nM) return;
    const int m0 = mblk * BM, n0 = nblk * BN;
    if constexpr (OUT == 0 && MODE == 0) {
        if (p.kslices > 1) {
            const size_t z = blockIdx.y;
            p.A += z * (size_t)p.K;
            p.W += z * (size_t)p.K;
            p.C += z * (size_t)p.M * (size_t)p.ldc;
        }
    }

    gemm2_tile_body<WM, WN, MODE, OUT, ABL, SCHED, WGM, KS_>(p, m0, n0, nblk, smem);
}


__global__ __launch_bounds__(256) void split2_kernel(const float* __restrict__ x, int ldx, unsigned short* __restrict__ y,
                                                     int ldy, size_t plane, int M, int N, float scale,
                                                     const float* __restrict__ scale_dev, int seq_out, int seq_in) {
    if (scale_dev) scale *= *scale_dev;
    const int c4n = ldy >> 2;
    const size_t total = (size_t)M * c4n;
    const bool wide_st = ldy % 8 == 0 && plane % 8 == 0 && ((uintptr_t)y & 15) == 0;
    for (size_t i = (size_t)blockIdx.x * 256 + threadIdx.x; i < total; i += (size_t)gridDim.x * 256) {
        const int row = (int)(i / c4n), c = (int)(i % c4n) * 4;
        int xrow = row;
        bool pad = false;
        if (seq_out > 0) {
            const int b = row / seq_out, t = row % seq_out;
            pad = t >= seq_in;
            xrow = b * seq_in + t;
        }
        float v[4] = {0.f, 0.f, 0.f, 0.f};
        if (pad) {
        } else if (c + 3 < N) {
            const float4 t = *reinterpret_cast<const float4*>(x + (size_t)xrow * ldx + c);
            v[0] = t.x; v[1] = t.y; v[2] = t.z; v[3] = t.w;
        } else {
#pragma unroll
            for (int e = 0; e < 4; ++e) if (c + e < N) v[e] = x[(size_t)xrow * ldx + c + e];
        }
        if (wide_st) store_split2x4_pair(y + (size_t)row * ldy + c, plane, v, scale, threadIdx.x);
        else store_split2x4(y + (size_t)row * ldy + c, plane, v, scale);
    }
}

__global__ __launch_bounds__(256) void absmax_kernel(const float* __restrict__ x, size_t n, unsigned* __restrict__ out) {
    float m = 0.f;
    for (size_t i = (size_t)blockIdx.x * 256 + threadIdx.x; i < n; i += (size_t)gridDim.x * 256) m = fmaxf(m, fabsf(x[i]));
    m = wave_max(m);
    if ((threadIdx.x & 63) == 0) atomicMax(out, __builtin_bit_cast(unsigned, m));
}

__global__ __launch_bounds__(256) void rowl1_bound_kernel(const float* __restrict__ W, int rows, int cols, int ld,
                                                          const float* __restrict__ bias, float in_bound, unsigned* __restrict__ out) {
    const int row = blockIdx.x * 4 + (threadIdx.x >> 6), lane = threadIdx.x & 63;
    if (row >= rows) return;
    float a = 0.f;
    for (int k = lane; k < cols; k += 64) a += fabsf(W[(size_t)row * ld + k]);
    a = wave_sum(a);
    const float bnd = (in_bound * a) * 1.0001f + (bias ? fabsf(bias[row]) : 0.f);
    if (lane == 0) atomicMax(out, __builtin_bit_cast(unsigned, bnd));
}

__global__ __launch_bounds__(256) void splitk_reduce_kernel(const float* __restrict__ part, int slices, size_t slice_stride, int M, int N,
                                                            const float* __restrict__ bias, int relu, const float* R1, int ldr1,
                                                            const float* R2, int ldr2, float* C, int ldc, unsigned short* C2, int ldc2,
                                                            size_t c_plane, float cscale) {
    const int n4 = N >> 2;
    const size_t total = (size_t)M * n4;
    for (size_t i = (size_t)blockIdx.x * 256 + threadIdx.x; i < total; i += (size_t)gridDim.x * 256) {
        const int row = (int)(i / n4), col = (int)(i % n4) * 4;
        const float* src = part + (size_t)row * N + col;
        float4 v = *reinterpret_cast<const float4*>(src);
        for (int z = 1; z < slices; ++z) {
            const float4 t = *reinterpret_cast<const float4*>(src + (size_t)z * slice_stride);
            v.x += t.x; v.y += t.y; v.z += t.z; v.w += t.w;
        }
        if (bias) {
            const float4 b = *reinterpret_cast<const float4*>(bias + col);
            v.x += b.x; v.y += b.y; v.z += b.z; v.w += b.w;
        }
        if (relu) { v.x = fmaxf(v.x, 0.f); v.y = fmaxf(v.y, 0.f); v.z = fmaxf(v.z, 0.f); v.w = fmaxf(v.w, 0.f); }
        if (R1) {
            const float4 r = *reinterpret_cast<const float4*>(R1 + (size_t)row * ldr1 + col);
            v.x = v.x + r.x; v.y = v.y + r.y; v.z = v.z + r.z; v.w = v.w + r.w;
        }
        if (R2) {
            const float4 r = *reinterpret_cast<const float4*>(R2 + (size_t)row * ldr2 + col);
            v.x = r.x + v.x; v.y = r.y + v.y; v.z = r.z + v.z; v.w = r.w + v.w;
        }
        if (C2) {
            const float o[4] = {v.x, v.y, v.z, v.w};
            store_split2x4(C2 + (size_t)row * ldc2 + col, c_plane, o, cscale);
        } else {
            *reinterpret_cast<float4*>(C + (size_t)row * ldc + col) = v;
        }
    }
}

template <int WM, int WN, int MODE, int OUT, int ABL = 0, int SCHED = 0, int WGM = 4, int KS_ = 32>
int launch_tile(const Gemm2Args& a, hipStream_t stream) {
    typedef Geo2<WM, WN, WGM, KS_> G;
    static PerDeviceOnce configured;
    if (!configured.done()) {
        PF_HIP_TRY(hipFuncSetAttribute(reinterpret_cast<const void*>(&gemm_f16x2_kernel<WM, WN, MODE, OUT, ABL, SCHED, WGM, KS_>),
                                       hipFuncAttributeMaxDynamicSharedMemorySize, G::LDS_B));
        configured.mark();
    }
    const int nM = ceil_div(a.M, G::BM), nN = ceil_div(a.N, G::BN);
    const int nMpad = (nM + 7) / 8 * 8;
    const unsigned gy = (OUT == 0 && MODE == 0 && a.kslices > 1) ? (unsigned)a.kslices : 1u;
    hipLaunchKernelGGL((gemm_f16x2_kernel<WM, WN, MODE, OUT, ABL, SCHED, WGM, KS_>), dim3((unsigned)nMpad * nN, gy), dim3(WGM * 128), G::LDS_B, stream, a, nM, nN);
    PF_HIP_TRY(hipGetLastError());
    return 0;
}
#if defined(PF_MEASUREMENT_KERNELS)
template <int MODE, int OUT>
int launch_pair(const Gemm2Args& a, hipStream_t stream) { return launch_tile<2, 4, MODE, OUT, 0, 0, 2, 16>(a, stream); }
template <int MODE, int OUT>
int launch_ring(const Gemm2Args& a, hipStream_t stream) { return launch_tile<2, 4, MODE, OUT, 0, 0, 4, 16>(a, stream); }
#endif
template <int MODE, int OUT>
int launch_one(const Gemm2Args& a, hipStream_t stream) {
    if constexpr (OUT == 1) {
        if (a.tile == 3) return launch_tile<2, 2, MODE, 1, 0, 0, 2>(a, stream);
    }
    if constexpr (OUT == 0) {
        if (a.tile == 3) return launch_tile<2, 2, MODE, 0, 0, 0, 2>(a, stream);
    }
#if defined(PF_MEASUREMENT_KERNELS)
    if constexpr (OUT == 0) {
        if (a.tile >= 256) return (a.tile >> 8) == 1 ? launch_tile<2, 4, MODE, 0, 0, 1>(a, stream) : launch_tile<2, 4, MODE, 0, 0, 2>(a, stream);
    }
    if constexpr (MODE == 0 && OUT == 0) {
        if (a.tile == 0x82) return launch_tile<2, 2, 0, 0, 2, 0, 2>(a, stream);
        if (a.tile == 0x83) return launch_tile<2, 2, 0, 0, 3, 0, 2>(a, stream);
        if (a.tile >= 16) {
            switch (a.tile >> 4) {
                case 1: return launch_tile<2, 4, 0, 0, 1>(a, stream);
                case 2: return launch_tile<2, 4, 0, 0, 2>(a, stream);
                case 3: return launch_tile<2, 4, 0, 0, 3>(a, stream);
                default: return launch_tile<2, 4, 0, 0, 4>(a, stream);
            }
        }
    }
#endif
    const int n_cu = device_cu_count();
    const long m_tiles = ceil_div(a.M, 256);
    const long wide_blocks = m_tiles * (a.N / 256), narrow_blocks = m_tiles * ceil_div(a.N, 128);
    const double cost_wide = (double)((wide_blocks + n_cu - 1) / n_cu), cost_narrow = 0.57 * (double)((narrow_blocks + n_cu - 1) / n_cu);
    const bool wide = a.tile == 2 || a.tile == 8 || a.tile == 9 || (a.tile == 0 && a.N % 256 == 0 && cost_wide <= cost_narrow);
    if constexpr (OUT == 0) {
        const long small_blocks = (long)ceil_div(a.M, 128) * ceil_div(a.N, 128);
        const double cost_small = 0.55 * (double)((small_blocks + 2 * n_cu - 1) / (2 * n_cu));
        if (a.tile == 0 && cost_small < (wide ? cost_wide : cost_narrow)) return launch_tile<2, 2, MODE, 0, 0, 0, 2>(a, stream);
    }
    if constexpr (OUT == 1) {
        if (a.tile == 0 && 2 * narrow_blocks <= n_cu) return launch_tile<2, 2, MODE, 1, 0, 0, 2>(a, stream);
    }
#if defined(PF_MEASUREMENT_KERNELS)
    if (wide && a.tile == 8) return launch_tile<2, 4, MODE, OUT, 0, 2>(a, stream);
    if (wide && a.tile == 9) return launch_tile<2, 4, MODE, OUT, 0, 3>(a, stream);
#endif
    return wide ? launch_tile<2, 4, MODE, OUT, 0, 0>(a, stream) : launch_tile<2, 2, MODE, OUT>(a, stream);
}

}

__global__ void pow2_scale_kernel(const float* __restrict__ amax, float* __restrict__ sc) {
    const float a = *amax;
    int e = a > 0.f ? (int)floorf(log2f(32768.f / a)) : 0;
    e = e > 100 ? 100 : (e < -100 ? -100 : e);
    sc[0] = ldexpf(1.f, e);
    sc[1] = ldexpf(1.f, -e);
}

int launch_pow2_scale(const float* amax_dev, float* sc, hipStream_t stream) {
    hipLaunchKernelGGL(pow2_scale_kernel, dim3(1), dim3(1), 0, stream, amax_dev, sc);
    PF_HIP_TRY(hipGetLastError());
    return 0;
}

__global__ void kv_scales_kernel(const float* __restrict__ amax, const float* __restrict__ lb, int n, float* __restrict__ out) {
    const int i = blockIdx.x * 64 + threadIdx.x;
    if (i >= 2 * n) return;
    const float bound = *amax * lb[2 * i] + lb[2 * i + 1];
    int e = bound > 0.f ? (int)floorf(log2f(32768.f / bound)) : 0;
    e = e > 60 ? 60 : (e < -60 ? -60 : e);
    out[4 * (i >> 1) + (i & 1)] = ldexpf(1.f, e);
    out[4 * (i >> 1) + 2 + (i & 1)] = ldexpf(1.f, -e);
}

int launch_kv_scales(const float* amax_dev, const float* l1_bmax_dev, int n_layers, float* out, hipStream_t stream) {
    hipLaunchKernelGGL(kv_scales_kernel, dim3(ceil_div(2 * n_layers, 64)), dim3(64), 0, stream, amax_dev, l1_bmax_dev, n_layers, out);
    PF_HIP_TRY(hipGetLastError());
    return 0;
}

int launch_split2(const float* x, int ldx, unsigned short* y, int ldy, size_t plane, int M, int N, float scale,
                  hipStream_t stream, const float* scale_dev, int seq_out, int seq_in) {
    PF_REQUIRE(M > 0 && N > 0 && ldy >= N && ldy % 4 == 0, "split2: ldy must cover N and be a multiple of 4");
    PF_REQUIRE(ldx % 4 == 0 && ((uintptr_t)x & 15) == 0 && ((uintptr_t)y & 7) == 0 && plane % 4 == 0, "split2: alignment");
    const size_t total = (size_t)M * (ldy >> 2);
    const unsigned blocks = (unsigned)((total + 255) / 256 < 8192 ? (total + 255) / 256 : 8192);
    hipLaunchKernelGGL(split2_kernel, dim3(blocks), dim3(256), 0, stream, x, ldx, y, ldy, plane, M, N, scale, scale_dev, seq_out, seq_in);
    PF_HIP_TRY(hipGetLastError());
    return 0;
}

int launch_absmax(const float* x, size_t n, float* out_dev, hipStream_t stream) {
    PF_HIP_TRY(hipMemsetAsync(out_dev, 0, sizeof(float), stream));
    const unsigned blocks = (unsigned)((n + 255) / 256 < 2048 ? (n + 255) / 256 : 2048);
    hipLaunchKernelGGL(absmax_kernel, dim3(blocks ? blocks : 1), dim3(256), 0, stream, x, n, reinterpret_cast<unsigned*>(out_dev));
    PF_HIP_TRY(hipGetLastError());
    return 0;
}

int launch_rowl1_bound(const float* W, int rows, int cols, int ld, const float* bias, float in_bound, float* out_dev,
                       hipStream_t stream) {
    PF_HIP_TRY(hipMemsetAsync(out_dev, 0, sizeof(float), stream));
    hipLaunchKernelGGL(rowl1_bound_kernel, dim3(ceil_div(rows, 4)), dim3(256), 0, stream, W, rows, cols, ld, bias, in_bound,
                       reinterpret_cast<unsigned*>(out_dev));
    PF_HIP_TRY(hipGetLastError());
    return 0;
}

static bool qkv_form_prefers_ps(const Gemm2Args& a) {
    static const int mode = [] { const char* e = getenv("PF_QKV_PS"); return e ? atoi(e) : 2; }();
    if (mode == 0 || !gemm_f16x2_ps_ok(a)) return false;
    if (mode == 1) return true;
    const int n_cu = device_cu_count();
    const long blocks = (long)ceil_div(a.M, 256) * (a.N / 256);
    if (blocks < n_cu) return false;
    const double rounds = (double)blocks / n_cu, whole = (double)((blocks + n_cu - 1) / n_cu);
    return whole / rounds > 1.15;
}

int gemm_f16x2_argmax_parts(int M, int N) { (void)M; return 2 * ceil_div(N, 256); }

int launch_gemm_f16x2(const Gemm2Args& a, hipStream_t stream) {
    PF_REQUIRE(a.M > 0 && a.N > 0 && a.K > 0, "gemm_f16x2: empty problem");
    if (a.ksplit > 1) {
        PF_REQUIRE((a.C || a.C2 || a.ln_g) && a.part && !a.amax_val && a.qkv_D <= 0 && a.a_kstep <= 0 && a.w_kstep <= 0 &&
                   a.K % (32 * a.ksplit) == 0 && a.N % 4 == 0 && ((uintptr_t)a.part & 15) == 0,
                   "gemm_f16x2: the split-K form needs K % (32 ksplit) == 0 and a partial buffer [ksplit][M][N]");
        if (a.C2) PF_REQUIRE(!a.ln_g && a.ldc2 % 4 == 0 && a.c_plane % 4 == 0 && ((uintptr_t)a.C2 & 7) == 0, "gemm_f16x2: split-K plane output alignment");
        else PF_REQUIRE((a.ln_g && !a.C) || (a.ldc % 4 == 0 && ((uintptr_t)a.C & 15) == 0), "gemm_f16x2: split-K output alignment");
        PF_REQUIRE(a.lda % 8 == 0 && a.ldw % 8 == 0 && a.a_plane % 8 == 0 && a.w_plane % 8 == 0 && ((uintptr_t)a.A & 15) == 0 &&
                   ((uintptr_t)a.W & 15) == 0 && (a.K / a.ksplit) % 8 == 0, "gemm_f16x2: operand alignment");
        if (a.bias) PF_REQUIRE(((uintptr_t)a.bias & 15) == 0, "gemm_f16x2: bias alignment");
        if (a.R1) PF_REQUIRE(a.ldr1 % 4 == 0 && ((uintptr_t)a.R1 & 15) == 0, "gemm_f16x2: R1 alignment");
        if (a.R2) PF_REQUIRE(a.ldr2 % 4 == 0 && ((uintptr_t)a.R2 & 15) == 0, "gemm_f16x2: R2 alignment");
        Gemm2Args p = a;
        p.ksplit = 0; p.kslices = a.ksplit; p.K = a.K / a.ksplit;
        p.C = a.part; p.ldc = a.N; p.C2 = nullptr; p.bias = nullptr; p.relu = 0; p.R1 = nullptr; p.R2 = nullptr; p.tile = 0;
        int rc = launch_tile<2, 2, 0, 0, 0, 0, 2>(p, stream);
        if (rc) return rc;
        if (a.ln_g) {
            PF_REQUIRE(a.ln_b && a.ln_y, "gemm_f16x2: the split-K + LayerNorm form needs beta and an output");
            return launch_splitk_reduce_ln(a.part, a.ksplit, (size_t)a.M * a.N, a.M, a.N, a.bias, a.relu, a.R1, a.ldr1, a.R2, a.ldr2, a.C, a.ldc, a.ln_g, a.ln_b,
                                           a.ln_eps, a.ln_y, a.ln_ldy, a.ln_out, a.ln_plane, a.ln_oscale, stream);
        }
        const size_t total = (size_t)a.M * (a.N >> 2);
        const unsigned blocks = (unsigned)((total + 255) / 256 < 4096 ? (total + 255) / 256 : 4096);
        hipLaunchKernelGGL(splitk_reduce_kernel, dim3(blocks), dim3(256), 0, stream, a.part, a.ksplit, (size_t)a.M * a.N, a.M, a.N,
                           a.bias, a.relu, a.R1, a.ldr1, a.R2, a.ldr2, a.C, a.ldc, a.C2, a.ldc2, a.c_plane, a.cscale);
        PF_HIP_TRY(hipGetLastError());
        return 0;
    }
    if (a.amax_val) {
        PF_REQUIRE(a.amax_idx && a.amax_ld >= gemm_f16x2_argmax_parts(a.M, a.N) && !a.R1 && !a.R2 && !a.relu && a.qkv_D <= 0,
                   "gemm_f16x2: the arg-max form takes bias only and needs amax_ld >= 2 ceil(N / 256)");
        PF_REQUIRE(a.K % 32 == 0 && a.lda % 8 == 0 && a.ldw % 8 == 0 && ((uintptr_t)a.A & 15) == 0 && ((uintptr_t)a.W & 15) == 0,
                   "gemm_f16x2: operand alignment");
        return launch_tile<2, 4, 0, 3, 0, 0>(a, stream);
    }
    PF_REQUIRE(a.K % 32 == 0, "gemm_f16x2: K must be a multiple of 32 (pad the planes with zeros)");
    PF_REQUIRE(a.lda % 8 == 0 && a.ldw % 8 == 0 && a.a_plane % 8 == 0 && a.w_plane % 8 == 0, "gemm_f16x2: operand strides % 8");
    PF_REQUIRE(((uintptr_t)a.A & 15) == 0 && ((uintptr_t)a.W & 15) == 0, "gemm_f16x2: operands must be 16-B aligned");
    PF_REQUIRE(a.N % 4 == 0, "gemm_f16x2: N % 4");
    if (a.C2 && a.qkv_D <= 0) PF_REQUIRE(a.ldc2 % 4 == 0 && a.c_plane % 4 == 0 && ((uintptr_t)a.C2 & 7) == 0, "gemm_f16x2: plane output alignment");
    else if (a.qkv_D <= 0 || a.C) PF_REQUIRE(a.C && a.ldc % 4 == 0 && ((uintptr_t)a.C & 15) == 0, "gemm_f16x2: output alignment");
    if (a.bias) PF_REQUIRE(((uintptr_t)a.bias & 15) == 0, "gemm_f16x2: bias alignment");
    if (a.R1) PF_REQUIRE(a.ldr1 % 4 == 0 && ((uintptr_t)a.R1 & 15) == 0, "gemm_f16x2: R1 alignment");
    if (a.R2) PF_REQUIRE(a.ldr2 % 4 == 0 && ((uintptr_t)a.R2 & 15) == 0, "gemm_f16x2: R2 alignment");
    const int mode = (a.R1 ? 1 : 0) | (a.R2 ? 2 : 0);
    if (a.qkv_D > 0) {
        PF_REQUIRE(mode == 0 && !a.relu && a.N == (a.kv_form ? 2 : 3) * a.qkv_D && a.qkv_D % 256 == 0 && a.M % 16 == 0,
                   "gemm_f16x2: the QKV / KV form needs N == 3 D (2 D), D % 256 == 0, M % 16 == 0, no residuals");
        PF_REQUIRE((a.kv_form || (a.Qp && a.C)) && a.Kp && a.VT && a.ldvt % 8 == 0 && a.vt_plane % 8 == 0 && a.qk_plane % 8 == 0 &&
                   ((uintptr_t)a.Qp & 15) == 0 && ((uintptr_t)a.Kp & 15) == 0 && ((uintptr_t)a.VT & 15) == 0,
                   "gemm_f16x2: QKV outputs");
    }
    if ((a.tile & 15) == 10 || (a.tile & 15) == 12) {
        if (gemm_f16x2_ps_ok(a)) return launch_gemm_f16x2_ps(a, stream);
// ... 89 lines not shown
```

### funasr_amd/ops.py

```python
from __future__ import annotations

import ctypes as C

import torch

from . import _lib


def _stream() -> int:
    return torch.cuda.current_stream().cuda_stream


def _ptr(t):
    return None if t is None else t.data_ptr()


def _f32c(t: torch.Tensor, name: str) -> torch.Tensor:
    if not t.is_cuda:
        raise RuntimeError(f"{name}: expected a tensor in GPU memory (there is no CPU path)")
    if t.dtype != torch.float32:
        raise TypeError(f"{name}: expected float32, got {t.dtype}")
    return t


# ... 473 lines not shown
                                  float(2.0 ** out_scale_exp), _ptr(yf), M, F | (int(abl) << 24) | (int(bool(w_kblocked)) << 28), int(time_iters), C.byref(ms), _stream()),
               "pf_k_ffn_f16x2")
    y = y2 if y2 is not None else yf
    return (c, y, float(ms.value)) if time_iters > 0 else (c, y)


def gemm_f16x2_row_fsmn(a2: torch.Tensor, w2: torch.Tensor, bias, v: torch.Tensor, taps: torch.Tensor, lo: torch.Tensor,
                        hi: torch.Tensor, add2=None, scale_exp: int = 0, ln=None, out_scale_exp: int = 0, ln_planes: bool = True,
                        want_c: bool = True, a_nt: bool = False, time_iters: int = 0, block_rows: int = 0):
    lib = _lib.load()
    assert a2.dtype == torch.float16 and w2.dtype == torch.float16 and a2.is_contiguous() and w2.is_contiguous()
    _, M, K = a2.shape
    assert w2.shape[1] == 512 and w2.shape[2] == K and M % 16 == 0 and ln is not None
    assert v.dtype == torch.float32 and v.shape == (M, 512) and v.stride(1) == 1 and taps.shape == (512, 11) and taps.is_contiguous()
    assert lo.dtype == torch.int32 and hi.dtype == torch.int32 and lo.numel() == M // 16 and hi.numel() == M // 16
    dev = a2.device
    c = torch.empty(M, 512, device=dev, dtype=torch.float32) if want_c else None
    g, b, eps = ln
    y2 = torch.empty(2, M, 512, device=dev, dtype=torch.float16) if ln_planes else None
    yf = None if ln_planes else torch.empty(M, 512, device=dev, dtype=torch.float32)
    ms = C.c_float(0)
    _lib.check(lib.pf_k_gemm_f16x2_row_fsmn(_ptr(a2), K, M * K, _ptr(w2), K, 512 * K, float(2.0 ** -scale_exp), _ptr(bias),
                                            _ptr(v), v.stride(0), _ptr(taps), _ptr(lo), _ptr(hi),
                                            _ptr(add2), add2.stride(0) if add2 is not None else 0, _ptr(c), 512, _ptr(g), _ptr(b),
                                            float(eps), _ptr(y2), M * 512, float(2.0 ** out_scale_exp), _ptr(yf), M, K,
                                            (int(a_nt) & 3) | (int(block_rows) << 8), int(time_iters), C.byref(ms), _stream()),
               "pf_k_gemm_f16x2_row_fsmn")
    y = y2 if y2 is not None else yf
    return (c, y, float(ms.value)) if time_iters > 0 else (c, y)


def layernorm_planes(x: torch.Tensor, gamma, beta, eps: float, scale_exp: int = 0, time_iters: int = 0):
    lib = _lib.load()
    M, D = x.shape
    assert x.stride(1) == 1
    y = torch.empty(2, M, D, device=x.device, dtype=torch.float16)
    ms = C.c_float(0)
    _lib.check(lib.pf_k_layernorm_planes(_ptr(x), x.stride(0), _ptr(gamma), _ptr(beta), _ptr(y), D, M * D, float(2.0 ** scale_exp),
                                         M, D, float(eps), int(time_iters), C.byref(ms), _stream()), "pf_k_layernorm_planes")
    return (y, float(ms.value)) if time_iters > 0 else y


def vt_columns(m: torch.Tensor) -> torch.Tensor:
    return (m & ~12) | ((m & 4) << 1) | ((m & 8) >> 1)


def gemm_f16x2_qkv(a2: torch.Tensor, w2: torch.Tensor, bias, D: int, scale_exp: int, q_mul: float, k_mul: float, v_mul: float,
                   kv_form: bool = False, tile: int = 0, time_iters: int = 0):
    lib = _lib.load()
    _, M, K = a2.shape
    dev = a2.device
    nseg = 2 if kv_form else 3
    assert w2.shape[1] == nseg * D and M % 16 == 0
    q2 = None if kv_form else torch.zeros(2, M + 32, D, device=dev, dtype=torch.float16)
    k2 = torch.zeros(2, M + 32, D, device=dev, dtype=torch.float16)
    v = None if kv_form else torch.empty(M, D, device=dev, dtype=torch.float32)
    ldvt = M + 64
    vt = torch.zeros(2, D, ldvt, device=dev, dtype=torch.float16)
    ms = C.c_float(0)
    _lib.check(lib.pf_k_gemm_f16x2_qkv(_ptr(a2), K, M * K, _ptr(w2), K, nseg * D * K, float(2.0 ** -scale_exp), _ptr(bias), M, D, K,
                                       int(kv_form), _ptr(q2), _ptr(k2), (M + 32) * D, _ptr(v), _ptr(vt), ldvt, D * ldvt,
                                       float(q_mul), float(k_mul), float(v_mul), int(tile), int(time_iters), C.byref(ms), _stream()),
               "pf_k_gemm_f16x2_qkv")
    out = dict(q2=q2, k2=k2, v=v, vt=vt)
    if time_iters > 0:
        out["ms"] = float(ms.value)
    return out


def gemm_f16x2_argmax(a2: torch.Tensor, w2: torch.Tensor, bias, scale_exp: int = 0) -> torch.Tensor:
    lib = _lib.load()
    _, M, K = a2.shape
    N = w2.shape[1]
    nparts = 2 * ((N + 255) // 256)
    dev = a2.device
    ids = torch.empty(M, device=dev, dtype=torch.int32)
    sval = torch.empty(M, nparts, device=dev, dtype=torch.float32)
    sidx = torch.empty(M, nparts, device=dev, dtype=torch.int32)
    _lib.check(lib.pf_k_gemm_f16x2_argmax(_ptr(a2), K, M * K, _ptr(w2), K, N * K, float(2.0 ** -scale_exp), _ptr(bias), M, N, K,
                                          _ptr(ids), _ptr(sval), _ptr(sidx), _stream()), "pf_k_gemm_f16x2_argmax")
    return ids


def attention_f16x2(q, k, v, klens, n_heads: int, scale: float, eq: int = 6, ek: int = 6, ev: int = 6, variant: int = 0,
                    time_iters: int = 0):
    lib = _lib.load()
    B, Tq, D = q.shape
    Tp = k.shape[1]
    assert Tp % 16 == 0 and D == n_heads * 128
    dev = q.device
    q2 = split2((q * scale).reshape(B * Tq, D).contiguous(), eq)
    k2 = torch.zeros(2, B * Tp + 32, D, device=dev, dtype=torch.float16)
    k2[:, : B * Tp] = split2(k.reshape(B * Tp, D).contiguous(), ek)
    v2 = split2(v.reshape(B * Tp, D).contiguous(), ev)
    col = vt_columns(torch.arange(B * Tp, device=dev))
    ldvt = B * Tp + 64
    vt = torch.zeros(2, D, ldvt, device=dev, dtype=torch.float16)
    vt[:, :, col] = v2.transpose(1, 2)
    o2 = torch.empty(2, B * Tq, D, device=dev, dtype=torch.float16)
    ms = C.c_float(0)
    _lib.check(lib.pf_k_attention_f16x2(_ptr(q2), B * Tq * D, _ptr(k2), (B * Tp + 32) * D, _ptr(vt), ldvt, D * ldvt, _ptr(o2), B * Tq * D,
                                        _ptr(klens), B, n_heads, Tp, Tq, float(2.0 ** -(eq + ek)), float(2.0 ** -10), int(variant),
                                        int(time_iters), C.byref(ms), _stream()), "pf_k_attention_f16x2")
    out = ((o2[0].float() + o2[1].float()) * 2.0 ** -ev).view(B, Tq, D)
    return (out, float(ms.value)) if time_iters > 0 else out


def attention_bf16(q, k, v, klens, n_heads: int, scale: float):
    lib = _lib.load()
    B, Tq, D = q.shape
    Tk = k.shape[1]
    assert q.dtype == torch.bfloat16 and q.stride(2) == 1 and k.stride(2) == 1 and v.stride(2) == 1
    out = torch.empty(B, Tq, D, device=q.device, dtype=torch.bfloat16)
    _lib.check(lib.pf_k_attention_bf16(_ptr(q), q.stride(1), _ptr(k), k.stride(1), _ptr(v), v.stride(1), _ptr(out), D,
                                       _ptr(klens), B, n_heads, Tq, Tk, float(scale), _stream()), "pf_k_attention_bf16")
    return out
```

### include/paraformer_hip.h

```cpp
#ifndef PARAFORMER_HIP_H_
#define PARAFORMER_HIP_H_

#include <stdint.h>

#ifdef __cplusplus
extern "C" {
#endif

#define PF_ABI_VERSION 5

const char* pf_last_error(void);
int pf_abi_version(void);
int pf_device_count(void);

int pf_set_concurrency_guard(int32_t on);
int pf_concurrency_guard(void);

typedef struct pf_frontend pf_frontend;

typedef struct pf_frontend_config {
    int32_t sample_rate;
    int32_t frame_length;
    int32_t frame_shift;
    int32_t n_mels;
// ... 350 lines not shown
int pf_stream_set_pe(pf_stream* s, const float* pe, int32_t rows);
int pf_stream_reset(pf_stream* s, void* stream);
int pf_stream_set_option(pf_stream* s, const char* key, int32_t value);
int pf_stream_step(pf_stream* s, const float* feats_dev, int32_t n_frames, int32_t is_final, int32_t tail_chunk,
                   int32_t* ids_host, int32_t* n_tokens_host, float* enc_out_dev, void* stream);
int pf_stream_step_begin(pf_stream* s, const float* feats_dev, int32_t n_frames, int32_t is_final, int32_t tail_chunk,
                         float* enc_out_dev, void* stream);
int pf_stream_step_end(pf_stream* s, int32_t* ids_host, int32_t* n_tokens_host);
int pf_stream_peek(pf_stream* s, float* cif_alpha_host, float* cif_hidden_host, int32_t* start_idx_host);

typedef struct pf_dp pf_dp;
int pf_dp_unique_id(void* id_out, int32_t cap);
pf_dp* pf_dp_create(const void* unique_id, int32_t id_bytes, int32_t world, int32_t rank);
int pf_dp_destroy(pf_dp* dp);
int pf_dp_world(const pf_dp* dp);
int pf_dp_rank(const pf_dp* dp);
int pf_dp_broadcast_encoder(pf_dp* dp, pf_encoder* e, int32_t root, void* stream);
int pf_dp_broadcast_predictor(pf_dp* dp, pf_predictor* p, int32_t root, void* stream);
int pf_dp_broadcast_decoder(pf_dp* dp, pf_decoder* d, int32_t root, void* stream);
int pf_dp_broadcast_ctc(pf_dp* dp, pf_ctc* c, int32_t root, void* stream);
int pf_dp_broadcast_raw(pf_dp* dp, void* buf_dev, int64_t bytes, int32_t root, void* stream);
int pf_dp_gather_ids(pf_dp* dp, const int32_t* ids_dev, int64_t count, int32_t* out_dev, int32_t root, void* stream);

int pf_frontend_fbank(pf_frontend* f, const float* wav_dev, int64_t n_samples, float* fbank_dev, void* stream);
int pf_frontend_lfr_cmvn(pf_frontend* f, const float* frames_dev, int32_t T, int32_t rows, float* out_dev, void* stream);

int pf_encoder_debug_poison(pf_encoder* e, int32_t byte);
int pf_decoder_debug_poison(pf_decoder* d, int32_t byte);
int pf_predictor_debug_poison(pf_predictor* p, int32_t byte);
int pf_k_gemm_skinny_ln(const float* A, int32_t lda, const float* W, int32_t ldw, const float* bias, const float* R2, int32_t ldr2,
                        float* Cout, int32_t ldc, int32_t M, int32_t N, int32_t K, int32_t relu, float* stats_out,
                        const float* stats_in, const float* ln_g, const float* ln_c, float ln_eps, const float* out_gamma, float* ws_part,
                        int32_t* ws_count, void* stream);
int pf_k_ln_consts(const float* W, int32_t ldw, int32_t N, int32_t K, const float* gamma, const float* beta, const float* bias, float* c,
                   void* stream);
int pf_set_skinny_max_m(int32_t m);
int pf_k_gemm_f32(const float* A, int32_t lda, const float* W, int32_t ldw, const float* bias, const float* R1,
                  int32_t ldr1, const float* R2, int32_t ldr2, float* C, int32_t ldc, int32_t M, int32_t N,
                  int32_t K, int32_t relu, void* stream);
int pf_measurement_build(void);
int pf_k_conv1d_gemm_f32(const float* hidden, const float* W, const float* bias, float* C, int32_t B, int32_t T, int32_t D,
                         int32_t N, int32_t taps, int32_t left, int32_t relu, const float* zero_dev, void* stream);
int pf_k_gemm_bf16(const void* A, int32_t lda, const void* W, int32_t ldw, const float* bias, const float* R1,
                   int32_t ldr1, const float* R2, int32_t ldr2, void* C, int32_t ldc, int32_t M, int32_t N, int32_t K,
                   int32_t relu, int32_t c_bf16, void* stream);
int pf_k_gemm_bf16_time(const void* A, int32_t lda, const void* W, int32_t ldw, const float* bias, void* C, int32_t ldc,
                        int32_t M, int32_t N, int32_t K, int32_t c_bf16, int32_t iters, float* ms_out, void* stream);
int pf_k_split3(const float* x, int32_t ldx, void* y3, int32_t ldy, int64_t plane, int32_t M, int32_t N, void* stream);
int pf_k_gemm_split3(const void* A3, int32_t lda, int64_t a_plane, const void* W3, int32_t ldw, int64_t w_plane,
                     const float* bias, const float* R1, int32_t ldr1, const float* R2, int32_t ldr2, float* C,
                     int32_t ldc, void* C3, int32_t ldc3, int64_t c_plane, int32_t M, int32_t N, int32_t K,
                     int32_t relu, int32_t iters, float* ms_out, void* stream);
int pf_k_gemm_f16x2_row(const void* A2, int32_t lda, int64_t a_plane, const void* W2, int32_t ldw, int64_t w_plane, float oscale,
                        const float* bias, const float* R1, int32_t ldr1, const float* R2, int32_t ldr2, float* C, int32_t ldc,
                        const float* ln_g, const float* ln_b, float ln_eps, void* Y2, int64_t y_plane, float yscale, float* Yf,
                        int32_t M, int32_t K, int32_t relu, int32_t a_nt, int32_t iters, float* ms_out, void* stream);
int pf_k_ffn_f16x2(const void* X2, const void* W1, const void* W2, const float* b1, const float* b2, float oscale1, float hscale,
                   float oscale2, const float* R, float* Cout, const float* ln_g, const float* ln_b, float ln_eps, void* Y2,
                   float yscale, float* Yf, int32_t M, int32_t F, int32_t iters, float* ms_out, void* stream);
int pf_k_gemm_f16x2_row_fsmn(const void* A2, int32_t lda, int64_t a_plane, const void* W2, int32_t ldw, int64_t w_plane, float oscale,
                             const float* bias, const float* fs_v, int32_t ldfv, const float* fs_w, const int32_t* fs_lo,
                             const int32_t* fs_hi, const float* R2, int32_t ldr2, float* C, int32_t ldc, const float* ln_g,
                             const float* ln_b, float ln_eps, void* Y2, int64_t y_plane, float yscale, float* Yf, int32_t M, int32_t K,
                             int32_t a_nt, int32_t iters, float* ms_out, void* stream);
int pf_k_layernorm_planes(const float* x, int32_t ldx, const float* gamma, const float* beta, void* y2, int32_t ldy, int64_t plane,
                          float scale, int32_t M, int32_t D, float eps, int32_t iters, float* ms_out, void* stream);
int pf_k_gemm_f16x2_qkv(const void* A2, int32_t lda, int64_t a_plane, const void* W2, int32_t ldw, int64_t w_plane, float oscale,
                        const float* bias, int32_t M, int32_t D, int32_t K, int32_t kv_form, void* Qp, void* Kp, int64_t qk_plane,
                        float* Vf, void* VT, int32_t ldvt, int64_t vt_plane, float q_mul, float k_mul, float v_mul, int32_t tile,
                        int32_t iters, float* ms_out, void* stream);
int pf_k_gemm_f16x2_argmax(const void* A2, int32_t lda, int64_t a_plane, const void* W2, int32_t ldw, int64_t w_plane, float oscale,
                           const float* bias, int32_t M, int32_t N, int32_t K, int32_t* ids, float* scratch_val,
                           int32_t* scratch_idx, void* stream);
int pf_k_split2(const float* x, int32_t ldx, void* y2, int32_t ldy, int64_t plane, int32_t M, int32_t N, float scale,
                void* stream);
int pf_k_gemm_f16x2(const void* A2, int32_t lda, int64_t a_plane, const void* W2, int32_t ldw, int64_t w_plane,
                    float oscale, const float* bias, const float* R1, int32_t ldr1, const float* R2, int32_t ldr2,
                    float* C, int32_t ldc, void* C2, int32_t ldc2, int64_t c_plane, float cscale, int32_t M, int32_t N,
                    int32_t K, int32_t relu, int32_t tile, int32_t iters, float* ms_out, void* stream);
int pf_k_attention_f16x2(const void* Q2, int64_t q_plane, const void* K2, int64_t k_plane, const void* VT2, int32_t ldvt,
                         int64_t vt_plane, void* O2, int64_t o_plane, const int32_t* klens_dev, int32_t B, int32_t H,
                         int32_t Tp, int32_t Tq, float sscale, float oscale, int32_t variant, int32_t iters, float* ms_out,
                         void* stream);
int pf_k_cast_bf16(const float* x, void* y, int64_t n, void* stream);
int pf_k_gemm_argmax_f32(const float* A, int32_t lda, const float* W, int32_t ldw, const float* bias, int32_t M,
                         int32_t N, int32_t K, int32_t* ids, float* scratch_val, int32_t* scratch_idx, void* stream);
int pf_k_log_softmax(const float* x, int32_t ldx, float* y, int32_t ldy, int32_t M, int32_t N, void* stream);
int pf_k_layernorm(const float* x, int32_t ldx, const float* gamma, const float* beta, float* y, int32_t ldy,
                   int32_t M, int32_t D, int32_t Dpad, float eps, void* stream);
int pf_k_fsmn(const float* in, int32_t ldin, const float* w, const float* R, int32_t ldr, float* out, int32_t ldo,
              const int32_t* lens_dev, int32_t B, int32_t T, int32_t C, int32_t K, int32_t left_pad, void* stream);
int pf_k_attention_f32(const float* Q, int32_t ldq, const float* K, int32_t ldk, const float* V, int32_t ldv,
                       float* O, int32_t ldo, const int32_t* klens_dev, int32_t B, int32_t H, int32_t Tq,
                       int32_t Tk, float scale, void* stream);
int pf_k_attention_f32_two_source(const float* Q, int32_t ldq, const float* K, int32_t ldk, const float* V, int32_t ldv,
                                  const float* K2, int32_t ldk2, const float* V2, int32_t ldv2, float* O, int32_t ldo,
                                  const int32_t* n1_dev, int32_t n1_stride, int32_t B, int32_t H, int32_t Tq,
                                  int32_t Tk, int32_t T2, int32_t n2, float scale, void* stream);
int pf_k_attention_small(const float* Q, int32_t ldq, const float* K, int32_t ldk, const float* V, int32_t ldv,
                         float* O, int32_t ldo, const int32_t* klens_dev, int32_t B, int32_t H, int32_t d_k,
                         int32_t Tq, int32_t Tk, float scale, void* stream);
int pf_k_gather_rows(const float* table, int32_t ld, int32_t rows, const int32_t* ids_dev, float* out, int32_t n,
                     int32_t D, void* stream);
int pf_k_attention_split3(const float* Q, int32_t ldq, const float* K, int32_t ldk, const float* V, int32_t ldv,
                          float* O, int32_t ldo, const int32_t* klens_dev, int32_t B, int32_t H, int32_t Tq,
                          int32_t Tk, float scale, void* stream);
int pf_k_attention_bf16(const void* Q, int32_t ldq, const void* K, int32_t ldk, const void* V, int32_t ldv, void* O,
                        int32_t ldo, const int32_t* klens_dev, int32_t B, int32_t H, int32_t Tq, int32_t Tk, float scale,
                        void* stream);
int pf_k_lstm(const float* x, const float* w_ih, const float* w_hh, const float* b_ih, const float* b_hh, int32_t B, int32_t T,
              int32_t D, int32_t H, int32_t ndir, float* out, void* stream);
int pf_k_cif(const float* alphas, const float* hidden, int32_t B, int32_t T, int32_t D, int32_t N, float* peaks,
             int32_t* n_fires, float* embeds, void* stream);
int pf_k_cif_tail(const float* alphas, const float* hidden, const int32_t* lens_host, int32_t B, int32_t T, int32_t D, int32_t N,
                  float tail_threshold, int32_t tail_mask, int32_t loop, float* alphas_out, float* peaks, int32_t* n_fires,
                  int32_t* n_tok, float* embeds, void* stream);
int pf_k_ctc_runs(const int32_t* ids_dev, const int32_t* lens_host, int32_t B, int32_t T, int32_t blank, int32_t* counts_dev,
                  int32_t* ranges_dev, int32_t ld, void* stream);
int pf_k_argmax_rows(const float* x, int32_t ldx, int32_t M, int32_t N, int32_t* ids, void* stream);
int pf_k_log_softmax_stats(const float* x, int32_t ldx, int32_t M, int32_t N, float* lse, int32_t* pred, void* stream);
int64_t pf_k_ctc_align_scratch_bytes(int32_t B, int32_t T_max, int32_t L_max);
int pf_k_ctc_align(const float* emis, int32_t ld, int32_t T, int32_t V, int32_t t0, const float* lse, const int32_t* pred,
                   const int32_t* targets_dev, int32_t ldt, const int32_t* in_lens_host, const int32_t* tgt_lens_host, int32_t B,
                   int32_t blank, int32_t* labels, int32_t T_out, void* scratch, int64_t scratch_bytes, void* stream);
int pf_k_gemm_f32_time(const float* A, int32_t lda, const float* W, int32_t ldw, const float* bias, float* C,
                       int32_t ldc, int32_t M, int32_t N, int32_t K, int32_t iters, float* ms_out, void* stream);

#ifdef __cplusplus
}
#endif
#endif
```

Measured before the change: 38000.

## Add four-wave cross-attention form and XCD-ordered job list for packed decoder rows

The decoder cross-attention kernel gains a 4-wave (128-query) workgroup variant. A host heuristic picks between 4 and 8 waves from how many scheduling rounds each form would need over the CUs. For packed variable-length token rows, a host-built job list uploaded with the offsets lets the grid cover only the query blocks that exist, grouped by XCD, instead of padded blocks that exit early. The absmax kernel is also vectorised with float4 loads and issues one atomic per block. In exchange this adds template instances, host work per call, and reliance on a round-cost constant.

```diff
diff --git a/funasr_amd/_lib.py b/funasr_amd/_lib.py
--- a/funasr_amd/_lib.py
+++ b/funasr_amd/_lib.py
@@ -292,6 +292,10 @@
                                   _f32, _i32, _i32, _i32, _i32, _i32, _i32, C.POINTER(C.c_float), _vp]),
     "pf_k_attention_f16x2": (C.c_int, [_vp, _i64, _vp, _i64, _vp, _i32, _i64, _vp, _i64, _vp, _i32, _i32, _i32, _i32, _f32, _f32,
                                        _i32, _i32, C.POINTER(C.c_float), _vp]),
+    "pf_k_attention_f16x2_packed": (C.c_int, [_vp, _i64, _vp, _i64, _vp, _i32, _i64, _vp, _i64, _vp, _vp, _i32, _i32, _i32, _i32, _f32,
+                                              _f32, _i32, _i32, C.POINTER(C.c_float), _vp]),
+    "pf_k_attention_f16x2_form": (C.c_int, [_pi32, _i32, _i32, _i32]),
+    "pf_k_absmax": (C.c_int, [_vp, _i64, _vp, _vp]),
     "pf_k_gemm_f16x2_row": (C.c_int, [_vp, _i32, _i64, _vp, _i32, _i64, _f32, _vp, _vp, _i32, _vp, _i32, _vp, _i32, _vp, _vp, _f32,
                                       _vp, _i64, _f32, _vp, _i32, _i32, _i32, _i32, _i32, C.POINTER(C.c_float), _vp]),
     "pf_k_gemm_skinny_ln": (C.c_int, [_vp, _i32, _vp, _i32, _vp, _vp, _i32, _vp, _i32, _i32, _i32, _i32, _i32, _vp, _vp, _vp, _vp, _f32, _vp, _vp, _vp, _vp]),
diff --git a/funasr_amd/csrc/attention_f16x2.hip b/funasr_amd/csrc/attention_f16x2.hip
--- a/funasr_amd/csrc/attention_f16x2.hip
+++ b/funasr_amd/csrc/attention_f16x2.hip
@@ -9,24 +9,30 @@
 constexpr int VP_B = DK * KT * 2;
 constexpr int STAGE_B = 2 * KP_B + 2 * VP_B;
 constexpr int OLD = DK + 4;
-constexpr int SLAB_B = 8 * 32 * OLD * 4;
-constexpr int LDS_BYTES = SLAB_B > 3 * STAGE_B ? SLAB_B : 3 * STAGE_B;
+constexpr int lds_bytes(int nstage, int waves) {
+    return waves * 32 * OLD * 4 > nstage * STAGE_B ? waves * 32 * OLD * 4 : nstage * STAGE_B;
+}
 constexpr float P_SCALE = 1024.f;
 typedef _Float16 f16x8 __attribute__((ext_vector_type(8)));
 
 constexpr float LAZY_TAU = 3.0f;
-template <int PIPE, bool LAZY = false>
-__global__ __launch_bounds__(512, 2) void attention_f16x2_kernel(Attn2Args p) {
+template <int PIPE, bool LAZY = false, int WAVES = 8, bool JOBS = false>
+__global__ __launch_bounds__(64 * WAVES, 2) void attention_f16x2_kernel(Attn2Args p) {
+    static_assert(WAVES == 8 || WAVES == 4, "attention_f16x2: 8 or 4 waves per workgroup");
     extern __shared__ __attribute__((aligned(16))) unsigned char smem[];
     constexpr int NSTAGE = PIPE ? 3 : 2;
-    constexpr int QB = 256;
-    constexpr int NV = 1;
+    constexpr int QB = 32 * WAVES;
+    constexpr int NV = 8 / WAVES;
 
     const int tid = threadIdx.x, lane = tid & 63;
     const int wave = __builtin_amdgcn_readfirstlane(tid >> 6);
     const int hh = lane >> 5, idx = lane & 31;
     int b, head, qblk;
-    if (p.xcd_nqb > 0) {
+    if constexpr (JOBS) {
+        const int job = p.jobs[blockIdx.x];
+        if (job < 0 || (job >> 12) >= p.B * p.H) return;
+        qblk = job & 4095; head = (job >> 12) % p.H; b = (job >> 12) / p.H;
+    } else if (p.xcd_nqb > 0) {
         const int L = blockIdx.x, j = L >> 3;
         const int pair = (j / p.xcd_nqb) * 8 + (L & 7);
         if (pair >= p.B * p.H) return;
@@ -241,39 +247,89 @@
                a.k_plane % 8 == 0 && a.vt_plane % 8 == 0 && a.o_plane % 8 == 0, "attention_f16x2: strides % 8");
     PF_REQUIRE(((uintptr_t)a.Q & 15) == 0 && ((uintptr_t)a.K & 15) == 0 && ((uintptr_t)a.VT & 15) == 0 && ((uintptr_t)a.O & 15) == 0,
                "attention_f16x2: 16-B alignment");
-    static PerDeviceOnce configured;
-    if (!configured.done()) {
-#if defined(PF_MEASUREMENT_KERNELS)
-        PF_HIP_TRY(hipFuncSetAttribute(reinterpret_cast<const void*>(&attention_f16x2_kernel<0>),
-                                       hipFuncAttributeMaxDynamicSharedMemorySize, LDS_BYTES));
-        PF_HIP_TRY(hipFuncSetAttribute(reinterpret_cast<const void*>(&attention_f16x2_kernel<1>),
-                                       hipFuncAttributeMaxDynamicSharedMemorySize, LDS_BYTES));
-#endif
-        PF_HIP_TRY(hipFuncSetAttribute(reinterpret_cast<const void*>(&attention_f16x2_kernel<0, true>),
-                                       hipFuncAttributeMaxDynamicSharedMemorySize, LDS_BYTES));
-        configured.mark();
-    }
-    const int rows = a.Tq > 0 ? a.Tq : a.Tp;
-    Attn2Args k = a;
+    PF_REQUIRE(a.waves == 0 || a.waves == 4 || a.waves == 8, "attention_f16x2: waves must be 0 (= 8), 4 or 8");
+    const int waves = a.waves == 4 ? 4 : 8;
 #if defined(PF_MEASUREMENT_KERNELS)
     PF_REQUIRE(a.variant == 0 || a.variant == 1 || a.variant == 3, "attention_f16x2: variant must be 0, 1 or 3");
 #else
     PF_REQUIRE(a.variant == 3, "attention_f16x2: variant must be 3 (variants 0 / 1: the measurement library, make measure)");
 #endif
-    const int nqb = ceil_div(rows, 256);
+    PF_REQUIRE(a.variant == 3 || waves == 8, "attention_f16x2: the four-wave form exists for variant 3 only");
+    constexpr int LDS8 = lds_bytes(2, 8), LDS8P = lds_bytes(3, 8), LDS4 = lds_bytes(2, 4);
+    static_assert(LDS8 == 135168 && LDS8P == 135168 && LDS4 == 67584 && 2 * LDS4 <= 163840, "attention_f16x2: LDS per workgroup");
+    static PerDeviceOnce configured;
+    if (!configured.done()) {
+#if defined(PF_MEASUREMENT_KERNELS)
+        PF_HIP_TRY(hipFuncSetAttribute(reinterpret_cast<const void*>(&attention_f16x2_kernel<0>),
+                                       hipFuncAttributeMaxDynamicSharedMemorySize, LDS8));
+        PF_HIP_TRY(hipFuncSetAttribute(reinterpret_cast<const void*>(&attention_f16x2_kernel<1>),
+                                       hipFuncAttributeMaxDynamicSharedMemorySize, LDS8P));
+#endif
+        PF_HIP_TRY(hipFuncSetAttribute(reinterpret_cast<const void*>(&attention_f16x2_kernel<0, true>),
+                                       hipFuncAttributeMaxDynamicSharedMemorySize, LDS8));
+        PF_HIP_TRY(hipFuncSetAttribute(reinterpret_cast<const void*>(&attention_f16x2_kernel<0, true, 4>),
+                                       hipFuncAttributeMaxDynamicSharedMemorySize, LDS4));
+        PF_HIP_TRY(hipFuncSetAttribute(reinterpret_cast<const void*>(&attention_f16x2_kernel<0, true, 8, true>),
+                                       hipFuncAttributeMaxDynamicSharedMemorySize, LDS8));
+        PF_HIP_TRY(hipFuncSetAttribute(reinterpret_cast<const void*>(&attention_f16x2_kernel<0, true, 4, true>),
+                                       hipFuncAttributeMaxDynamicSharedMemorySize, LDS4));
+        configured.mark();
+    }
+    const int rows = a.Tq > 0 ? a.Tq : a.Tp;
+    Attn2Args k = a;
+    const int nqb = ceil_div(rows, 32 * waves);
     dim3 grid(nqb, a.H, a.B);
     k.xcd_nqb = (a.xcd_nqb >= 0 && nqb > 1) ? nqb : 0;
     if (k.xcd_nqb > 0) grid = dim3((unsigned)(ceil_div(a.B * a.H, 8) * 8 * nqb), 1, 1);
-    if (a.variant == 3)
-        hipLaunchKernelGGL((attention_f16x2_kernel<0, true>), grid, dim3(512), LDS_BYTES, stream, k);
+    if (a.jobs) {
+        PF_REQUIRE(a.variant == 3 && a.qoffs && a.n_jobs > 0 && a.n_jobs % 8 == 0 && nqb <= 4096, "attention_f16x2: a job list needs qoffs, a multiple of 8 jobs and at most 4096 query blocks");
+        k.xcd_nqb = 0;
+        grid = dim3((unsigned)a.n_jobs, 1, 1);
+    }
+    if (a.variant == 3 && waves == 4 && a.jobs)
+        hipLaunchKernelGGL((attention_f16x2_kernel<0, true, 4, true>), grid, dim3(256), LDS4, stream, k);
+    else if (a.variant == 3 && waves == 4)
+        hipLaunchKernelGGL((attention_f16x2_kernel<0, true, 4>), grid, dim3(256), LDS4, stream, k);
+    else if (a.variant == 3 && a.jobs)
+        hipLaunchKernelGGL((attention_f16x2_kernel<0, true, 8, true>), grid, dim3(512), LDS8, stream, k);
+    else if (a.variant == 3)
+        hipLaunchKernelGGL((attention_f16x2_kernel<0, true>), grid, dim3(512), LDS8, stream, k);
 #if defined(PF_MEASUREMENT_KERNELS)
     else if (a.variant == 1)
-        hipLaunchKernelGGL(attention_f16x2_kernel<1>, grid, dim3(512), LDS_BYTES, stream, k);
+        hipLaunchKernelGGL(attention_f16x2_kernel<1>, grid, dim3(512), LDS8P, stream, k);
     else
-        hipLaunchKernelGGL(attention_f16x2_kernel<0>, grid, dim3(512), LDS_BYTES, stream, k);
+        hipLaunchKernelGGL(attention_f16x2_kernel<0>, grid, dim3(512), LDS8, stream, k);
 #endif
     PF_HIP_TRY(hipGetLastError());
     return 0;
 }
 
-}
+constexpr double XATTN_ROUND_COST_4 = 1.05;
+int attention_f16x2_waves(const int32_t* q_lens, int B, int H, int n_cu, int force) {
+    if (force == 4 || force == 8) return force;
+    if (!q_lens || B <= 0 || H <= 0 || n_cu <= 0) return 8;
+    long jobs8 = 0, jobs4 = 0;
+    for (int b = 0; b < B; ++b) {
+        const int n = q_lens[b] > 0 ? q_lens[b] : 0;
+        jobs8 += (long)H * ceil_div(n, 256);
+        jobs4 += (long)H * ceil_div(n, 128);
+    }
+    const long rounds8 = (jobs8 + n_cu - 1) / n_cu, rounds4 = (jobs4 + 2L * n_cu - 1) / (2L * n_cu);
+    return (double)rounds4 * XATTN_ROUND_COST_4 < (double)rounds8 ? 4 : 8;
+}
+
+void attention_f16x2_jobs(const int32_t* q_lens, int B, int H, int waves, std::vector<int32_t>& out) {
+    const int QB = waves == 4 ? 128 : 256;
+    std::vector<int32_t> xcd[8];
+    for (int pair = 0; pair < B * H; ++pair) {
+        const int n = q_lens[pair / H] > 0 ? q_lens[pair / H] : 0;
+        for (int qblk = 0; qblk < ceil_div(n, QB) && qblk < 4096; ++qblk) xcd[pair & 7].push_back((int32_t)(pair << 12 | qblk));
+    }
+    size_t len = 1;
+    for (const auto& x : xcd) len = x.size() > len ? x.size() : len;
+    out.assign(len * 8, -1);
+    for (int x = 0; x < 8; ++x)
+        for (size_t i = 0; i < xcd[x].size(); ++i) out[i * 8 + x] = xcd[x][i];
+}
+
+}
diff --git a/funasr_amd/csrc/common.h b/funasr_amd/csrc/common.h
--- a/funasr_amd/csrc/common.h
+++ b/funasr_amd/csrc/common.h
@@ -3,6 +3,7 @@
 #include <stdint.h>
 #include <stdio.h>
 #include <string>
+#include <vector>
 #include <atomic>
 
 typedef float floatx16 __attribute__((ext_vector_type(16)));
@@ -383,8 +384,12 @@
     const int* qoffs;
     int xcd_nqb;
     const int* koffs;
+    int waves;
+    const int* jobs; int n_jobs;
 };
 int launch_attention_f16x2(const Attn2Args& a, hipStream_t stream);
+int attention_f16x2_waves(const int32_t* q_lens, int B, int H, int n_cu, int force = 0);
+void attention_f16x2_jobs(const int32_t* q_lens, int B, int H, int waves, std::vector<int32_t>& out);
 
 int launch_asf_scores(const float* Q, int ldq, const float* K, int ldk, float* P_scratch, float* out, int H, int dk, int N, int T,
                       int klen, float scale, hipStream_t stream);
diff --git a/funasr_amd/csrc/engine_decoder.hip b/funasr_amd/csrc/engine_decoder.hip
--- a/funasr_amd/csrc/engine_decoder.hip
+++ b/funasr_amd/csrc/engine_decoder.hip
@@ -448,6 +448,7 @@
     }
     bool pack = false;
     const int* offs_dev = nullptr;
+    int xattn_waves = 8, xattn_njobs = 0;
     if (may_pack) {
         int total = 0;
         d->h_offs.assign((size_t)B + 1, 0);
@@ -456,9 +457,17 @@
         if (total > 0 && total < Mq_pad) {
             d->h_map.resize((size_t)total);
             for (int b = 0; b < B; ++b) for (int t = 0; t < tok_lens[b]; ++t) d->h_map[(size_t)d->h_offs[b] + t] = b * N + t;
-            if (d->offs_dev.ensure(sizeof(int32_t) * ((size_t)B + 1)) || d->map_dev.ensure(sizeof(int32_t) * (size_t)Mq_pad) ||
+            const char* ew = getenv("PF_XATTN_WAVES");
+            const char* ej = getenv("PF_XATTN_JOBS");
+            xattn_waves = attention_f16x2_waves(tok_lens, B, c.n_heads, device_cu_count(), ew ? atoi(ew) : 0);
+            if ((long)B * c.n_heads < (1L << 19) && !(ej && atoi(ej) == 0)) {
+                attention_f16x2_jobs(tok_lens, B, c.n_heads, xattn_waves, d->h_jobs);
+                d->h_offs.insert(d->h_offs.end(), d->h_jobs.begin(), d->h_jobs.end());
+                xattn_njobs = (int)d->h_jobs.size();
+            }
+            if (d->offs_dev.ensure(sizeof(int32_t) * d->h_offs.size()) || d->map_dev.ensure(sizeof(int32_t) * (size_t)Mq_pad) ||
                 d->ids_packed.ensure(sizeof(int32_t) * (size_t)Mq_pad)) return -2;
-            if (upload_h2d(d->offs_dev.p, d->h_offs.data(), sizeof(int32_t) * ((size_t)B + 1), s) ||
+            if (upload_h2d(d->offs_dev.p, d->h_offs.data(), sizeof(int32_t) * d->h_offs.size(), s) ||
                 upload_h2d(d->map_dev.p, d->h_map.data(), sizeof(int32_t) * (size_t)total, s)) return -2;
             if ((rc = launch_gather_rows(embeds, D, Mq_pad, d->map_dev.as<int>(), x, total, D, s))) return rc;
             pack = true; offs_dev = d->offs_dev.as<int>(); Mq = total;
@@ -470,6 +479,12 @@
             return -2;
         if ((rc = launch_split3(memory, D, d->mem16.as<unsigned short>(), D, (size_t)Mk * D, Mk, D, s))) return rc;
         mem3 = d->mem16.as<unsigned short>();
+    }
+    const int* xattn_jobs = xattn_njobs > 0 ? offs_dev + B + 1 : nullptr;
+    if (x2 && !pack) {
+        const char* ew = getenv("PF_XATTN_WAVES");
+        std::vector<int32_t> padded((size_t)B, N);
+        xattn_waves = attention_f16x2_waves(padded.data(), B, c.n_heads, device_cu_count(), ew ? atoi(ew) : 0);
     }
     DecRows rows{x2 ? 3 : x3 ? 2 : 0, Mq, B, N, offs_dev, (c.kernel_size - 1) / 2 + (c.sanm_shift > 0 ? c.sanm_shift : 0), s};
     for (int l = 0; l < c.n_blocks; ++l) {
@@ -515,6 +530,7 @@
                 aa.klens = d->mem_lens.as<int>(); aa.B = B; aa.H = c.n_heads; aa.Tp = Tp; aa.Tq = N; aa.qoffs = offs_dev;
                 aa.sscale = pow2f(-w.e_q); aa.sscale_dev = lsc + 2; aa.oscale = pow2f(-10);
                 aa.variant = 3;
+                aa.waves = xattn_waves; aa.jobs = xattn_jobs; aa.n_jobs = xattn_njobs;
                 ProfScope ps(PROF_ATTN, 4.0 * tok_mem * D, s);
                 if ((rc = launch_attention_f16x2(aa, s))) return rc;
             }
diff --git a/funasr_amd/csrc/engine_internal.h b/funasr_amd/csrc/engine_internal.h
--- a/funasr_amd/csrc/engine_internal.h
+++ b/funasr_amd/csrc/engine_internal.h
@@ -471,7 +471,7 @@
     int e_an = 0;
     DevBuf asf_p;
     DevBuf offs_dev, map_dev, ids_packed;
-    std::vector<int32_t> h_offs, h_map;
+    std::vector<int32_t> h_offs, h_map, h_jobs;
 };
 
 
diff --git a/funasr_amd/csrc/engine_kernels.hip b/funasr_amd/csrc/engine_kernels.hip
--- a/funasr_amd/csrc/engine_kernels.hip
+++ b/funasr_amd/csrc/engine_kernels.hip
@@ -147,35 +147,56 @@
     *ms_out = ms / iters;
     return 0;
 }
-int pf_k_attention_f16x2(const void* Q2, int64_t q_plane, const void* K2, int64_t k_plane, const void* VT2, int32_t ldvt,
-                         int64_t vt_plane, void* O2, int64_t o_plane, const int32_t* klens_dev, int32_t B, int32_t H,
-                         int32_t Tp, int32_t Tq, float sscale, float oscale, int32_t variant, int32_t iters, float* ms_out,
-                         void* stream) {
-    hipStream_t s = reinterpret_cast<hipStream_t>(stream);
+static int k_attention_f16x2(const void* Q2, int64_t q_plane, const void* K2, int64_t k_plane, const void* VT2, int32_t ldvt,
+                             int64_t vt_plane, void* O2, int64_t o_plane, const int32_t* klens_dev, const int32_t* qoffs_dev,
+                             int32_t B, int32_t H, int32_t Tp, int32_t Tq, float sscale, float oscale, int32_t variant,
+                             int32_t iters, float* ms_out, void* stream) {
+    hipStream_t s = reinterpret_cast<hipStream_t>(stream);
+    PF_REQUIRE((variant & ~255) == 0 && (variant & 96) != 96 && (!(variant & 128) || qoffs_dev), "pf_k_attention_f16x2: variant bits");
     Attn2Args aa{};
     const int D = H * 128;
     aa.Q = reinterpret_cast<const unsigned short*>(Q2); aa.ldq = D; aa.q_plane = (size_t)q_plane;
     aa.K = reinterpret_cast<const unsigned short*>(K2); aa.ldk = D; aa.k_plane = (size_t)k_plane;
     aa.VT = reinterpret_cast<const unsigned short*>(VT2); aa.ldvt = ldvt; aa.vt_plane = (size_t)vt_plane;
     aa.O = reinterpret_cast<unsigned short*>(O2); aa.ldo = D; aa.o_plane = (size_t)o_plane;
-    aa.klens = klens_dev; aa.B = B; aa.H = H; aa.Tp = Tp; aa.Tq = Tq; aa.sscale = sscale; aa.oscale = oscale;
+    aa.klens = klens_dev; aa.B = B; aa.H = H; aa.Tp = Tp; aa.Tq = Tq; aa.sscale = sscale; aa.oscale = oscale; aa.qoffs = qoffs_dev;
     aa.variant = variant & 15; aa.xcd_nqb = (variant & 16) ? -1 : 0;
-    int rc;
+    aa.waves = (variant & 32) ? 4 : (variant & 64) ? 8 : 0;
+    static DevBuf jobs_dev;
+    if (variant & 128) {
+        std::vector<int32_t> offs((size_t)B + 1), jobs;
+        PF_HIP_TRY(hipStreamSynchronize(s));
+        PF_HIP_TRY(hipMemcpy(offs.data(), qoffs_dev, sizeof(int32_t) * offs.size(), hipMemcpyDeviceToHost));
+        for (int b = 0; b < B; ++b) offs[b] = offs[b + 1] - offs[b];
+        attention_f16x2_jobs(offs.data(), B, H, aa.waves == 4 ? 4 : 8, jobs);
+        if (jobs_dev.ensure(sizeof(int32_t) * jobs.size())) return -2;
+        PF_HIP_TRY(hipMemcpy(jobs_dev.p, jobs.data(), sizeof(int32_t) * jobs.size(), hipMemcpyHostToDevice));
+        aa.jobs = jobs_dev.as<int>(); aa.n_jobs = (int)jobs.size();
+    }
     if (iters <= 0 || !ms_out) return launch_attention_f16x2(aa, s);
-    for (int i = 0; i < 3; ++i) if ((rc = launch_attention_f16x2(aa, s))) return rc;
-    hipEvent_t a, b;
-    PF_HIP_TRY(hipEventCreate(&a));
-    PF_HIP_TRY(hipEventCreate(&b));
-    PF_HIP_TRY(hipEventRecord(a, s));
-    for (int i = 0; i < iters; ++i) if ((rc = launch_attention_f16x2(aa, s))) return rc;
-    PF_HIP_TRY(hipEventRecord(b, s));
-    PF_HIP_TRY(hipEventSynchronize(b));
-    float ms = 0.f;
-    PF_HIP_TRY(hipEventElapsedTime(&ms, a, b));
-    (void)hipEventDestroy(a);
-    (void)hipEventDestroy(b);
-    *ms_out = ms / iters;
-    return 0;
+    return time_launches([&] { return launch_attention_f16x2(aa, s); }, iters, ms_out, s);
+}
+int pf_k_attention_f16x2(const void* Q2, int64_t q_plane, const void* K2, int64_t k_plane, const void* VT2, int32_t ldvt,
+                         int64_t vt_plane, void* O2, int64_t o_plane, const int32_t* klens_dev, int32_t B, int32_t H,
+                         int32_t Tp, int32_t Tq, float sscale, float oscale, int32_t variant, int32_t iters, float* ms_out,
+                         void* stream) {
+    return k_attention_f16x2(Q2, q_plane, K2, k_plane, VT2, ldvt, vt_plane, O2, o_plane, klens_dev, nullptr, B, H, Tp, Tq, sscale,
+                             oscale, variant, iters, ms_out, stream);
+}
+int pf_k_attention_f16x2_packed(const void* Q2, int64_t q_plane, const void* K2, int64_t k_plane, const void* VT2, int32_t ldvt,
+                                int64_t vt_plane, void* O2, int64_t o_plane, const int32_t* klens_dev, const int32_t* qoffs_dev,
+                                int32_t B, int32_t H, int32_t Tp, int32_t Tq, float sscale, float oscale, int32_t variant,
+                                int32_t iters, float* ms_out, void* stream) {
+    PF_REQUIRE(qoffs_dev && Tq > 0, "pf_k_attention_f16x2_packed: qoffs_dev and Tq");
+    return k_attention_f16x2(Q2, q_plane, K2, k_plane, VT2, ldvt, vt_plane, O2, o_plane, klens_dev, qoffs_dev, B, H, Tp, Tq, sscale,
+                             oscale, variant, iters, ms_out, stream);
+}
+int pf_k_absmax(const float* x, int64_t n, float* out_dev, void* stream) {
+    PF_REQUIRE(x && out_dev && n > 0, "pf_k_absmax: null/empty");
+    return launch_absmax(x, (size_t)n, out_dev, reinterpret_cast<hipStream_t>(stream));
+}
+int pf_k_attention_f16x2_form(const int32_t* q_lens, int32_t B, int32_t H, int32_t n_cu) {
+    return attention_f16x2_waves(q_lens, B, H, n_cu, 0);
 }
 int pf_k_gemm_f16x2_row(const void* A2, int32_t lda, int64_t a_plane, const void* W2, int32_t ldw, int64_t w_plane, float oscale,
                         const float* bias, const float* R1, int32_t ldr1, const float* R2, int32_t ldr2, float* C, int32_t ldc,
diff --git a/funasr_amd/csrc/gemm_f16x2.hip b/funasr_amd/csrc/gemm_f16x2.hip
--- a/funasr_amd/csrc/gemm_f16x2.hip
+++ b/funasr_amd/csrc/gemm_f16x2.hip
@@ -310,10 +310,33 @@
 }
 
 __global__ __launch_bounds__(256) void absmax_kernel(const float* __restrict__ x, size_t n, unsigned* __restrict__ out) {
+    __shared__ float wmax[4];
+    const size_t head = n < 4 ? n : (size_t)((16 - ((uintptr_t)x & 15)) & 15) >> 2;
+    const size_t n4 = (n - head) >> 2, tail0 = head + 4 * n4;
+    const float4* __restrict__ x4 = reinterpret_cast<const float4*>(x + head);
+    const size_t stride = (size_t)gridDim.x * 256;
     float m = 0.f;
-    for (size_t i = (size_t)blockIdx.x * 256 + threadIdx.x; i < n; i += (size_t)gridDim.x * 256) m = fmaxf(m, fabsf(x[i]));
+    size_t i = (size_t)blockIdx.x * 256 + threadIdx.x;
+    for (; i + 3 * stride < n4; i += 4 * stride) {
+        const float4 a = x4[i], b = x4[i + stride], c = x4[i + 2 * stride], d = x4[i + 3 * stride];
+        m = fmaxf(m, fmaxf(fmaxf(fabsf(a.x), fabsf(a.y)), fmaxf(fabsf(a.z), fabsf(a.w))));
+        m = fmaxf(m, fmaxf(fmaxf(fabsf(b.x), fabsf(b.y)), fmaxf(fabsf(b.z), fabsf(b.w))));
+        m = fmaxf(m, fmaxf(fmaxf(fabsf(c.x), fabsf(c.y)), fmaxf(fabsf(c.z), fabsf(c.w))));
+        m = fmaxf(m, fmaxf(fmaxf(fabsf(d.x), fabsf(d.y)), fmaxf(fabsf(d.z), fabsf(d.w))));
+    }
+    for (; i < n4; i += stride) {
+        const float4 a = x4[i];
+        m = fmaxf(m, fmaxf(fmaxf(fabsf(a.x), fabsf(a.y)), fmaxf(fabsf(a.z), fabsf(a.w))));
+    }
+    if (blockIdx.x == 0) {
+        if (threadIdx.x < head) m = fmaxf(m, fabsf(x[threadIdx.x]));
+        if (tail0 + threadIdx.x < n) m = fmaxf(m, fabsf(x[tail0 + threadIdx.x]));
+    }
     m = wave_max(m);
-    if ((threadIdx.x & 63) == 0) atomicMax(out, __builtin_bit_cast(unsigned, m));
+    if ((threadIdx.x & 63) == 0) wmax[threadIdx.x >> 6] = m;
+    __syncthreads();
+    if (threadIdx.x == 0)
+        atomicMax(out, __builtin_bit_cast(unsigned, fmaxf(fmaxf(wmax[0], wmax[1]), fmaxf(wmax[2], wmax[3]))));
 }
 
 __global__ __launch_bounds__(256) void rowl1_bound_kernel(const float* __restrict__ W, int rows, int cols, int ld,
@@ -475,7 +498,7 @@
 
 int launch_absmax(const float* x, size_t n, float* out_dev, hipStream_t stream) {
     PF_HIP_TRY(hipMemsetAsync(out_dev, 0, sizeof(float), stream));
-    const unsigned blocks = (unsigned)((n + 255) / 256 < 2048 ? (n + 255) / 256 : 2048);
+    const unsigned blocks = (unsigned)((n + 1023) / 1024 < 512 ? (n + 1023) / 1024 : 512);
     hipLaunchKernelGGL(absmax_kernel, dim3(blocks ? blocks : 1), dim3(256), 0, stream, x, n, reinterpret_cast<unsigned*>(out_dev));
     PF_HIP_TRY(hipGetLastError());
     return 0;
diff --git a/funasr_amd/ops.py b/funasr_amd/ops.py
--- a/funasr_amd/ops.py
+++ b/funasr_amd/ops.py
@@ -579,14 +579,9 @@
     return ids
 
 
-def attention_f16x2(q, k, v, klens, n_heads: int, scale: float, eq: int = 6, ek: int = 6, ev: int = 6, variant: int = 0,
-                    time_iters: int = 0):
-    lib = _lib.load()
-    B, Tq, D = q.shape
-    Tp = k.shape[1]
-    assert Tp % 16 == 0 and D == n_heads * 128
-    dev = q.device
-    q2 = split2((q * scale).reshape(B * Tq, D).contiguous(), eq)
+def _attention_f16x2_kv(k, v, ek: int, ev: int):
+    B, Tp, D = k.shape
+    dev = k.device
     k2 = torch.zeros(2, B * Tp + 32, D, device=dev, dtype=torch.float16)
     k2[:, : B * Tp] = split2(k.reshape(B * Tp, D).contiguous(), ek)
     v2 = split2(v.reshape(B * Tp, D).contiguous(), ev)
@@ -594,13 +589,61 @@
     ldvt = B * Tp + 64
     vt = torch.zeros(2, D, ldvt, device=dev, dtype=torch.float16)
     vt[:, :, col] = v2.transpose(1, 2)
+    return k2, vt, ldvt
+
+
+def attention_f16x2(q, k, v, klens, n_heads: int, scale: float, eq: int = 6, ek: int = 6, ev: int = 6, variant: int = 0,
+                    time_iters: int = 0, return_planes: bool = False):
+    lib = _lib.load()
+    B, Tq, D = q.shape
+    Tp = k.shape[1]
+    assert Tp % 16 == 0 and D == n_heads * 128
+    dev = q.device
+    q2 = split2((q * scale).reshape(B * Tq, D).contiguous(), eq)
+    k2, vt, ldvt = _attention_f16x2_kv(k, v, ek, ev)
     o2 = torch.empty(2, B * Tq, D, device=dev, dtype=torch.float16)
     ms = C.c_float(0)
     _lib.check(lib.pf_k_attention_f16x2(_ptr(q2), B * Tq * D, _ptr(k2), (B * Tp + 32) * D, _ptr(vt), ldvt, D * ldvt, _ptr(o2), B * Tq * D,
                                         _ptr(klens), B, n_heads, Tp, Tq, float(2.0 ** -(eq + ek)), float(2.0 ** -10), int(variant),
                                         int(time_iters), C.byref(ms), _stream()), "pf_k_attention_f16x2")
-    out = ((o2[0].float() + o2[1].float()) * 2.0 ** -ev).view(B, Tq, D)
+    out = o2 if return_planes else ((o2[0].float() + o2[1].float()) * 2.0 ** -ev).view(B, Tq, D)
     return (out, float(ms.value)) if time_iters > 0 else out
+
+
+def attention_f16x2_packed(q_rows, qoffs, k, v, klens, n_heads: int, scale: float, eq: int = 6, ek: int = 6, ev: int = 6,
+                           variant: int = 3, o2=None, time_iters: int = 0):
+    lib = _lib.load()
+    R, D = q_rows.shape
+    B, Tp, _ = k.shape
+    assert Tp % 16 == 0 and D == n_heads * 128 and qoffs.dtype == torch.int32 and qoffs.numel() == B + 1
+    offs = qoffs.cpu().tolist()
+    assert 0 <= offs[0] and offs[-1] <= R and all(a <= b for a, b in zip(offs, offs[1:]))
+    Tq = max(1, max(b - a for a, b in zip(offs, offs[1:])))
+    q2 = split2((q_rows * scale).contiguous(), eq)
+    k2, vt, ldvt = _attention_f16x2_kv(k, v, ek, ev)
+    if o2 is None:
+        o2 = torch.zeros(2, R, D, device=q_rows.device, dtype=torch.float16)
+    assert o2.shape == (2, R, D) and o2.dtype == torch.float16 and o2.is_contiguous()
+    ms = C.c_float(0)
+    _lib.check(lib.pf_k_attention_f16x2_packed(_ptr(q2), R * D, _ptr(k2), (B * Tp + 32) * D, _ptr(vt), ldvt, D * ldvt, _ptr(o2), R * D,
+                                               _ptr(klens), _ptr(qoffs), B, n_heads, Tp, Tq, float(2.0 ** -(eq + ek)),
+                                               float(2.0 ** -10), int(variant), int(time_iters), C.byref(ms), _stream()),
+               "pf_k_attention_f16x2_packed")
+    return (o2, float(ms.value)) if time_iters > 0 else o2
+
+
+def absmax(x: torch.Tensor) -> torch.Tensor:
+    lib = _lib.load()
+    assert x.dtype == torch.float32 and x.is_contiguous() and x.numel() > 0
+    out = torch.empty(1, device=x.device, dtype=torch.float32)
+    _lib.check(lib.pf_k_absmax(_ptr(x), x.numel(), _ptr(out), _stream()), "pf_k_absmax")
+    return out
+
+
+def attention_f16x2_form(q_lens, n_heads: int, n_cu: int) -> int:
+    lib = _lib.load()
+    arr = (C.c_int32 * len(q_lens))(*[int(n) for n in q_lens])
+    return int(lib.pf_k_attention_f16x2_form(arr, len(q_lens), int(n_heads), int(n_cu)))
 
 
 def attention_bf16(q, k, v, klens, n_heads: int, scale: float):
diff --git a/include/paraformer_hip.h b/include/paraformer_hip.h
--- a/include/paraformer_hip.h
+++ b/include/paraformer_hip.h
@@ -456,6 +456,12 @@
                          int64_t vt_plane, void* O2, int64_t o_plane, const int32_t* klens_dev, int32_t B, int32_t H,
                          int32_t Tp, int32_t Tq, float sscale, float oscale, int32_t variant, int32_t iters, float* ms_out,
                          void* stream);
+int pf_k_attention_f16x2_packed(const void* Q2, int64_t q_plane, const void* K2, int64_t k_plane, const void* VT2, int32_t ldvt,
+                                int64_t vt_plane, void* O2, int64_t o_plane, const int32_t* klens_dev, const int32_t* qoffs_dev,
+                                int32_t B, int32_t H, int32_t Tp, int32_t Tq, float sscale, float oscale, int32_t variant,
+                                int32_t iters, float* ms_out, void* stream);
+int pf_k_absmax(const float* x, int64_t n, float* out_dev, void* stream);
+int pf_k_attention_f16x2_form(const int32_t* q_lens, int32_t B, int32_t H, int32_t n_cu);
 int pf_k_cast_bf16(const float* x, void* y, int64_t n, void* stream);
 int pf_k_gemm_argmax_f32(const float* A, int32_t lda, const float* W, int32_t ldw, const float* bias, int32_t M,
                          int32_t N, int32_t K, int32_t* ids, float* scratch_val, int32_t* scratch_idx, void* stream);
```

Result: no change. 38250, median of 6 (+0.7%).
